# LiqunZhao/Neural-ordinary-differential-equations-based-Lyapunov-Barrier-Actor-Critic-NLBAC

Measured on AMD Instinct MI355X. Metric: ODE-integrate+update samples/sec, Unicycle batch 4096, higher is better.
Workload: dtype f32; 1 GPU; Unicycle B=4096 dopri5 (BASELINE.json configs[1] at B=4096 dopri5); NODE fit on 32768 rows every 10 updates; replay of 65536 synthetic transitions resident in HBM; solver=dopri5, adjoint=False, batch_per_gpu=4096, global_batch=4096, node_fit_rows_per_gpu=32768, parallelism=dp1, hipgraph=False

## Files before the change

include/nlbac_hip.h:

```cpp
#ifndef NLBAC_HIP_H
#define NLBAC_HIP_H

#ifdef __cplusplus
extern "C" {
#endif

#define NLBAC_ABI_VERSION 17
#define NLBAC_MAX_LAYERS 6
#define NLBAC_MAX_NETS 8
#define NLBAC_MLP_TILE 32

typedef void *nlbac_stream_t;

int nlbac_abi_version(void);
const char *nlbac_last_error(void);
int nlbac_elect_selftest(float *partials, unsigned *ticket, float *out, int n_blocks, int n_vals, unsigned salt,
                         nlbac_stream_t s);

typedef struct nlbac_mlp {
    int n_layers, in_dim, hid, out_dim;
    const float *params;
    int w_off[NLBAC_MAX_LAYERS];
    int b_off[NLBAC_MAX_LAYERS];
    float *packed;
    int pf_off[NLBAC_MAX_LAYERS];
    int pb_off[NLBAC_MAX_LAYERS];
    int rr_fwd_off, rr_bwd_off, packed_floats;
    int rr_kind;
} nlbac_mlp;

typedef struct nlbac_mlp_io {
    const float *x0; int x0_dim, x0_ld;
    const float *x1; int x1_dim, x1_ld;
    float *y; int y_ld;
    float *acts;
    long acts_ls;
    const float *dy; int dy_ld;
    int dz_first;
    float *dz;
    float *dx; int dx_ld;
    int dx_first;
    float *grad;
    float *skinny_ws;
    unsigned *masks;
} nlbac_mlp_io;

int nlbac_mlp_masks_ok(const nlbac_mlp *nets, int n_nets);

int nlbac_mlp_pack_layout(nlbac_mlp *net );
int nlbac_mlp_pack(const nlbac_mlp *nets, int n_nets, nlbac_stream_t s);

int nlbac_mlp_fwd(const nlbac_mlp *nets, const nlbac_mlp_io *io, int n_nets, int B, nlbac_stream_t s);
typedef struct nlbac_gauss_head {
    const float *eps, *scale, *bias; int n_u;
    float *action; int action_ld; float *logp;
    int cf_kind, cf_net, cf_nh;
    const float *cf_ps, *cf_ps_next, *cf_V, *cf_hazards;
    float cf_r2, cf_dt, cf_gamma_b, cf_gamma_l;
    float *cf_matr, *cf_bmatr, *cf_partials; unsigned *cf_tickets;
    int cf_n_cbf, cf_n_clf; float cf_batch_size; int cf_do_lambda_update, cf_do_backup_lambda_update, cf_ratio_mode, cf_backup_mode;
    float cf_lam_lo, cf_lam_hi;
    float *cf_sc;
    int cf_defer; unsigned *cf_tiles;
} nlbac_gauss_head;
int nlbac_mlp_fwd_gauss(const nlbac_mlp *nets, const nlbac_mlp_io *io, int n_nets, int B,
                        const nlbac_gauss_head *head, nlbac_stream_t s);
int nlbac_mlp_fwd_head_ok(const nlbac_mlp *nets, int n_nets);
int nlbac_mlp_fwd_head(const nlbac_mlp *nets, const nlbac_mlp_io *io, int n_nets, int B,
                       const nlbac_gauss_head *head, nlbac_stream_t s);
int nlbac_mlp_bwd_data(const nlbac_mlp *nets, const nlbac_mlp_io *io, int n_nets, int B, nlbac_stream_t s);
struct nlbac_dy_head;
int nlbac_mlp_bwd_data_head(const nlbac_mlp *nets, const nlbac_mlp_io *io, int n_nets, int B,
                            const struct nlbac_dy_head *head, nlbac_stream_t s);
long nlbac_mlp_bwd_weights_ws_floats(const nlbac_mlp *nets, int n_nets, int B);
int nlbac_mlp_bwd_weights(const nlbac_mlp *nets, const nlbac_mlp_io *io, int n_nets, int B,
                          int n_slabs, long slab_stride, float *ws, long ws_floats, nlbac_stream_t s);

int nlbac_adam_prepare(void *state, double lr, nlbac_stream_t s);
int nlbac_adam_step(float *p, float *m, float *v, const float *grad, int n_slabs, long slab_stride,
                    long n, const void *state, float *target, float tau, nlbac_stream_t s);
int nlbac_adam_fused(float *p, float *m, float *v, const float *grad, int n_slabs, long slab_stride, long n,
                     void *state, double lr, float *target, float tau, const void *scatter,
                     const void *scatter_target, int scatter_slots ,
                     int n_alpha ,
                     const long *alpha_off, float *const *alpha_dst,
                     const float *mirror_src, float *mirror_dst ,
                     int n_mirror, nlbac_stream_t s);
int nlbac_reduce_slabs(float *out, const float *grad, int n_slabs, long slab_stride, long n, nlbac_stream_t s);
int nlbac_soft_update(float *target, const float *src, long n, float tau, nlbac_stream_t s);

int nlbac_gauss_sample_fwd(const float *heads, int heads_ld, const float *eps, const float *scale,
                           const float *bias, int n_u, int n, float *action, int action_ld,
                           float *logp, nlbac_stream_t s);
int nlbac_gauss_sample_bwd(const float *heads, int heads_ld, const float *eps, const float *scale,
                           int n_u, int n, int rows_per_problem, const float *da0, int da0_ld,
                           const float *da1, int da1_ld, const float *da2, int da2_ld,
                           const float *alpha, float dlogp_mul, float *dheads, int dheads_ld,
                           nlbac_stream_t s);

#define NLBAC_SC_SIZE 128

int nlbac_td_targets(const float *q1t, const float *q2t, const float *lt, const float *nlogp,
                     const float *reward, const float *constraint, const float *mask, int rcm_ld,
                     const float *q1, const float *q2, const float *lf, const float *alpha,
                     float gamma, int B, int B_norm, float *dq1, float *dq2, float *dlf, float *next_q,
                     float *next_l, float *partials, unsigned *ticket, float mul, float *out, nlbac_stream_t s);

typedef struct nlbac_actor_scalar_args {
    float target_entropy;
    const float *log_alpha[2];
    float *g_log_alpha[2];
    float *sc;
} nlbac_actor_scalar_args;
int nlbac_actor_q_terms(const float *q1, const float *q2, const float *logp, const float *alpha,
                        int B, int B_norm, int P, float *dq1, float *dq2, float *partials,
                        const nlbac_actor_scalar_args *fused, unsigned *ticket, nlbac_stream_t s);
typedef struct nlbac_auglag_args {
    int n_cbf, n_clf;
    float batch_size;
    int do_lambda_update, do_backup_lambda_update, ratio_mode, backup_mode;
    float lam_lo, lam_hi;
} nlbac_auglag_args;
typedef struct nlbac_head_sums {
    int kind;
    int n_nets;
    const float *partials;
    const unsigned *n_tiles;
    float mul; float *out; float *out_x;
    int B_norm; nlbac_actor_scalar_args actor;
    float *sc;
} nlbac_head_sums;
typedef struct nlbac_dy_head {
    int kind, B_norm;
    const float *heads; int heads_ld; const float *eps; const float *scale; int n_u;
    const float *da[3]; int da_ld[3];
    const float *alpha;
    float dlogp_mul; float *dheads; int dheads_ld;
    const float *q1t, *q2t, *lt, *nlogp, *reward, *constraint, *mask; int rcm_ld;
    const float *q[3]; float gamma; float *dq[3]; float *next_q, *next_l;
    const float *xt, *xsig; int xsig_ld; const float *xq; float *dxq; float *out_x;
    const float *qa, *qb, *logp; float *dqa, *dqb; int n_prob;
    nlbac_actor_scalar_args actor;
    float *partials; unsigned *ticket; float mul; float *out;
    int cb_kind, cb_nh;
    const float *cb_ps_next, *cb_matr, *cb_bmatr, *cb_hazards, *cb_sc;
    float cb_dt, cb_batch;
    float *cb_dps_next, *cb_dV;
    int sums_defer; unsigned *sums_tiles;
    nlbac_head_sums finish[3];
    int cb_defer; const float *cb_partials; const unsigned *cb_tiles; nlbac_auglag_args cb_auglag; float *cb_stage;
} nlbac_dy_head;
int nlbac_actor_scalars(const float *partials, int n_blk, int B, int first_problem, int P, float target_entropy,
                        const float *log_alpha, int log_alpha_stride, float *g_log_alpha, float *sc,
                        nlbac_stream_t s);
int nlbac_alpha_refresh(const float *log_alpha, int log_alpha_stride, int first_problem, int P, float *sc,
                        nlbac_stream_t s);

int nlbac_unicycle_state(const float *obs, int obs_ld, int B, float l_p,
                         float *state ,
                         int n_copies, float *ps , nlbac_stream_t s);
int nlbac_unicycle_lookahead(const float *x , int n, float l_p, float *ps , nlbac_stream_t s);
int nlbac_unicycle_lookahead_bwd(const float *x, const float *dps, const float *dps2 , int n,
                                 float l_p, float *dx , nlbac_stream_t s);

int nlbac_unicycle_constraints_fwd(const float *ps, const float *ps_next, const float *V,
                                   const float *V_next, const float *hazards, int n_hz, float r_coll,
                                   float dt, float gamma_b, float gamma_l, int B, float *matr,
                                   float *bmatr, float *partials, const nlbac_auglag_args *fused,
                                   unsigned *ticket, float *sc, nlbac_stream_t s);
int nlbac_auglag(const float *partials, int n_blk, int n_cbf, int n_clf, float batch_size,
                 int do_lambda_update, int do_backup_lambda_update ,
                 int ratio_mode, int backup_mode, float lam_lo, float lam_hi, float *sc, nlbac_stream_t s);
int nlbac_unicycle_constraints_bwd(const float *ps_next, const float *matr, const float *bmatr,
                                   const float *hazards, int n_hz, float dt, float batch_size, int B,
                                   const float *sc, float *dps_next, float *dV_next, nlbac_stream_t s);

int nlbac_cars_state(const float *obs, int obs_ld, int n, float *state, nlbac_stream_t s);
int nlbac_cars_rollout_inputs(const float *mb, int ld, int t_col, int nt_col, const float *pi2, int B,
                              float *state, float *y0_2, float *c1, float *c2, nlbac_stream_t s);
int nlbac_cars_obs(const float *state, int n, float *obs, nlbac_stream_t s);
int nlbac_cars_constraints_fwd(const float *state, const float *x1, const float *x2, const float *V,
                               const float *V1, float gamma_b, float gamma_l, float radius, int B,
                               float *matr, float *bmatr, float *partials, const nlbac_auglag_args *fused,
                               unsigned *ticket, float *sc, nlbac_stream_t s);
int nlbac_cars_constraints_bwd(const float *matr, const float *bmatr, float gamma_b, float batch_size, int B,
                               const float *sc, float *dx1, float *dx2, float *dV1, nlbac_stream_t s);
int nlbac_add_cols(float *dst, int dst_ld, int col0, const float *src, int src_ld, int ncols, int n,
                   nlbac_stream_t s);
int nlbac_add_cols_plus(float *dst, int ld, int col0, const float *src, int src_ld, int ncols, int n_src,
                        const float *add, int n, nlbac_stream_t s);

int nlbac_td_value(const float *next_target, const float *signal, int sig_ld, const float *mask, int mask_ld,
                   const float *pred, float gamma, int B, int B_norm, float *dpred, float *next_out ,
                   float *partials, unsigned *ticket, float mul, float *out, nlbac_stream_t s);
int nlbac_unicycle_obs_fwd(const float *x , int n, float goal_x, float goal_y, float *obs, int obs_ld,
                           nlbac_stream_t s);
int nlbac_unicycle_obs_bwd(const float *x, const float *dobs, int dobs_ld, int n, float goal_x, float goal_y,
                           float *dx , int accumulate, nlbac_stream_t s);
int nlbac_barrier_constraints_fwd(const float *Bv, const float *Bn, const float *V, const float *Vn, float dt,
                                  float gamma_b, float gamma_l, int B, float *matr, float *partials,
                                  const nlbac_auglag_args *fused, unsigned *ticket, float *sc, nlbac_stream_t s);
int nlbac_barrier_constraints_bwd(const float *matr, float dt, float batch_size, int B, const float *sc,
                                  float *dBn, float *dVn, nlbac_stream_t s);

int nlbac_pvtol_state(const float *obs, int obs_ld, int n, float *st6, float *op , nlbac_stream_t s);
int nlbac_pvtol_obs_fwd(const float *x6, const float *op_prev, int op_rows, float follow, float goal_x, float goal_y,
                        int n, float *obs, int obs_ld, float *op_out , nlbac_stream_t s);
int nlbac_pvtol_obs_bwd(const float *x6, const float *dobs, int dobs_ld, float follow, float goal_x, float goal_y,
                        int n, float *dx, int accumulate, nlbac_stream_t s);
int nlbac_pvtol_constraints_fwd(const float *st6, const float *op0, const float *x1, const float *x2, const float *x3,
                                const float *V, const float *V1, const float *hazards, int n_hz, float r_coll,
                                float d_op, float y_max, float y_min, float follow, float gamma_b, float gamma_l,
                                int B, int NP, float *matr, float *bmatr, float *partials,
                                const nlbac_auglag_args *fused, unsigned *ticket, float *sc, nlbac_stream_t s);
int nlbac_pvtol_constraints_bwd(const float *matr, const float *bmatr, const float *x1, const float *x2,
                                const float *x3, const float *hazards, int n_hz, float follow, float gamma_b,
                                float batch_size, int B, int NP, const float *sc, float *dx1, float *dx2, float *dx3,
                                float *dV1, nlbac_stream_t s);

int nlbac_mse_fwd_bwd(const float *pred, int pred_ld, const float *target, int target_ld, int n, int n_norm,
                      int d, float *dpred, int dpred_ld, float *partials, nlbac_stream_t s);

int nlbac_affine_combine_fwd(const float *f, const float *g, const float *u, int n_s, int n_u, int n,
                             float *k, nlbac_stream_t s);
int nlbac_affine_combine_bwd(const float *dk, const float *g, const float *u, int n_s, int n_u, int n,
                             float mul, float *dg, float *du, int accumulate_du, nlbac_stream_t s);
int nlbac_rk_combine(const float *y0, const float *K, int n_k, const float *coef, const float *h_host,
                     const double *h_dev, int h_dev_stride, int P, int rows_per_problem, int n_s,
                     float *out, nlbac_stream_t s);
int nlbac_rk_stage_bwd(const float *dYup, const float *dXf, const float *dXg, int dx_ld, int n_k,
                       const float *coef, const float *h_host, const double *h_dev, int h_dev_stride,
                       int P, int rows_per_problem, int n_s, float *dK, float *dy0, int accumulate_dy0,
                       float *du_ext , int n_ext,
                       nlbac_stream_t s);
typedef struct nlbac_rk_chain {
    const double *ctl;
    long slot_floats;
    int norm_mode;
    int n_slots;
    float rtol, atol;
    double t_end;
    float *partials;
    unsigned *tickets;
    double *ctl_w;
    double *hslots;
    double *alog;
    int alog_cap;
    double *ctl_host;
    float *interp_out;
    int interp_kind; float interp_l; float *interp_p;
    int interp_bwd;
    const float *interp_dout, *interp_dp, *interp_dp2, *interp_x;
    double ctl_seq;
    int norm_defer, norm_pre;
    const float *partials_pre;
} nlbac_rk_chain;
int nlbac_rk_interp_ok(const nlbac_mlp *f, const nlbac_mlp *g);
typedef struct nlbac_in_map {
    int kind;
    const float *obs; int obs_ld;
    float l;
    float *ps;
} nlbac_in_map;
int nlbac_node_rk_fwd(const nlbac_mlp *f, const nlbac_mlp *g, const float *y0, const float *u, int P,
                      int rows_per_problem, int stage_begin, int stage_end, int n_stages_total,
                      const float *beta, const float *c_out, int n_out, const float *c_err, int n_err,
                      const float *h_host, const double *h_dev, int h_dev_stride, float *K, float *Y,
                      float *G, float *acts_f, long acts_f_ls, float *acts_g, long acts_g_ls, int acts_bits,
                      float *out, float *err, const nlbac_rk_chain *chain,
                      const nlbac_in_map *in_map , nlbac_stream_t s);
int nlbac_node_rk_mask_words(const nlbac_mlp *f, const nlbac_mlp *g, int which);
int nlbac_node_rk_bwd(const nlbac_mlp *f, const nlbac_mlp *g, const float *u, const float *G, int P,
                      int rows_per_problem, int n_stages_total, int st_lo, int st_hi, int dx_stage0,
                      const float *beta, const float *h_host, const double *h_dev, int h_dev_stride,
                      const float *acts_f, long acts_f_ls, const float *acts_g, long acts_g_ls,
                      int acts_bits ,
                      float *dz_f, float *dz_g, float *dG, float *dK, const float *dYup, float *dy0,
                      int dy0_in, float *du, int du_acc, const nlbac_rk_chain *chain, int back_idx,
                      nlbac_stream_t s);
int nlbac_node_rk_traj_ok(const nlbac_mlp *f, const nlbac_mlp *g);
int nlbac_node_rk_traj_fwd(const nlbac_mlp *f, const nlbac_mlp *g, const float *x0, const float *u, int n, int H,
                           int n_stages, const float *beta, const float *c_out, float h, float *out, float *K, float *Y,
                           float *G, float *acts_f, long acts_f_ls, float *acts_g, long acts_g_ls, int acts_bits,
                           nlbac_stream_t s);
int nlbac_node_rk_traj_bwd(const nlbac_mlp *f, const nlbac_mlp *g, const float *u, int n, int H, int n_stages,
                           const float *beta, const float *c_out, float h, const float *G, const float *acts_f,
                           long acts_f_ls, const float *acts_g, long acts_g_ls, int acts_bits, const float *dout,
                           float *dx0, float *du, float *dK, float *dG, float *dz_f, float *dz_g, nlbac_stream_t s);
int nlbac_concat_rk_traj_ok(const nlbac_mlp *net);
int nlbac_concat_rk_traj_fwd(const nlbac_mlp *net, const float *x0, const float *c, int n, int H, int n_stages,
                             const float *beta, const float *c_out, float h, float *out, float *Xin, float *acts,
                             long acts_ls, int acts_bits, const float *norm, nlbac_stream_t s);
int nlbac_concat_rk_traj_bwd(const nlbac_mlp *net, int n, int H, int n_stages, const float *beta, const float *c_out,
                             float h, const float *acts, long acts_ls, int acts_bits, const float *norm,
                             const float *dout, float *dx0, float *dc, float *dK, float *dz, nlbac_stream_t s);
int nlbac_node_rk_grid_fwd(const nlbac_mlp *f, const nlbac_mlp *g, const float *x0, const float *u, int n, int H,
                           int n_stages, const float *beta, const float *c_out, const float *hs, const float *hs_host,
                           float *out, float *K, float *Y, float *G, float *acts_f, long acts_f_ls, float *acts_g,
                           long acts_g_ls, int acts_bits, nlbac_stream_t s);
int nlbac_node_rk_grid_bwd(const nlbac_mlp *f, const nlbac_mlp *g, const float *u, int n, int H, int n_stages,
                           const float *beta, const float *c_out, const float *hs, const float *hs_host,
                           const float *G, const float *acts_f, long acts_f_ls, const float *acts_g, long acts_g_ls,
                           int acts_bits, const float *dout, float *dx0, float *du, float *dK, float *dG, float *dz_f,
                           float *dz_g, nlbac_stream_t s);
int nlbac_concat_rk_grid_fwd(const nlbac_mlp *net, const float *x0, const float *c, int n, int H, int n_stages,
                             const float *beta, const float *c_out, const float *hs, const float *hs_host, float *out,
                             float *Xin, float *acts, long acts_ls, int acts_bits, const float *norm, nlbac_stream_t s);
int nlbac_concat_rk_grid_bwd(const nlbac_mlp *net, int n, int H, int n_stages, const float *beta, const float *c_out,
                             const float *hs, const float *hs_host, const float *acts, long acts_ls, int acts_bits,
                             const float *norm, const float *dout, float *dx0, float *dc, float *dK, float *dz,
                             nlbac_stream_t s);
int nlbac_node_rk_subgrid_fwd(const nlbac_mlp *f, const nlbac_mlp *g, const float *x0, const float *u, int n, int H,
                              int n_stages, const float *beta, const float *c_out, const float *hs,
                              const float *hs_host, const int *ofs, const int *ofs_host, const float *theta,
                              const float *theta_host, int T, float *out, float *K, float *Y, float *G, float *acts_f,
                              long acts_f_ls, float *acts_g, long acts_g_ls, int acts_bits, nlbac_stream_t s);
int nlbac_node_rk_subgrid_bwd(const nlbac_mlp *f, const nlbac_mlp *g, const float *u, int n, int H, int n_stages,
                              const float *beta, const float *c_out, const float *hs, const float *hs_host,
                              const int *ofs, const int *ofs_host, const float *theta, const float *theta_host, int T,
                              const float *G, const float *acts_f, long acts_f_ls, const float *acts_g, long acts_g_ls,
                              int acts_bits, const float *dout, float *dx0, float *du, float *dK, float *dG,
                              float *dz_f, float *dz_g, nlbac_stream_t s);
int nlbac_concat_rk_subgrid_fwd(const nlbac_mlp *net, const float *x0, const float *c, int n, int H, int n_stages,
                                const float *beta, const float *c_out, const float *hs, const float *hs_host,
                                const int *ofs, const int *ofs_host, const float *theta, const float *theta_host, int T,
                                float *out, float *Xin, float *acts, long acts_ls, int acts_bits, const float *norm,
                                nlbac_stream_t s);
int nlbac_concat_rk_subgrid_bwd(const nlbac_mlp *net, int n, int H, int n_stages, const float *beta, const float *c_out,
                                const float *hs, const float *hs_host, const int *ofs, const int *ofs_host,
                                const float *theta, const float *theta_host, int T, const float *acts, long acts_ls,
                                int acts_bits, const float *norm, const float *dout, float *dx0, float *dc, float *dK,
                                float *dz, nlbac_stream_t s);
int nlbac_node_rk_hold_fwd(const nlbac_mlp *f, const nlbac_mlp *g, const float *x0, const float *u, int n, int H,
                           int n_stages, const float *beta, const float *c_out, const float *hs, const float *hs_host,
                           int m, float *out, float *K, float *Y, float *G, float *acts_f, long acts_f_ls,
                           float *acts_g, long acts_g_ls, int acts_bits, nlbac_stream_t s);
int nlbac_node_rk_hold_bwd(const nlbac_mlp *f, const nlbac_mlp *g, const float *u, int n, int H, int n_stages,
                           const float *beta, const float *c_out, const float *hs, const float *hs_host, int m,
                           const float *G, const float *acts_f, long acts_f_ls, const float *acts_g, long acts_g_ls,
                           int acts_bits, const float *dout, float *dx0, float *du, float *dK, float *dG, float *dz_f,
                           float *dz_g, nlbac_stream_t s);
int nlbac_concat_rk_hold_fwd(const nlbac_mlp *net, const float *x0, const float *c, int n, int H, int n_stages,
                             const float *beta, const float *c_out, const float *hs, const float *hs_host, int m,
                             float *out, float *Xin, float *acts, long acts_ls, int acts_bits, const float *norm,
                             nlbac_stream_t s);
int nlbac_concat_rk_hold_bwd(const nlbac_mlp *net, int n, int H, int n_stages, const float *beta, const float *c_out,
                             const float *hs, const float *hs_host, int m, const float *acts, long acts_ls,
                             int acts_bits, const float *norm, const float *dout, float *dx0, float *dc, float *dK,
                             float *dz, nlbac_stream_t s);
int nlbac_concat_rk_fwd(const nlbac_mlp *net, const float *y0, const float *c, int P, int rows_per_problem,
                        int stage_begin, int stage_end, int n_stages_total, const float *beta,
                        const float *c_out, int n_out, const float *c_err, int n_err, const float *h_host,
                        const double *h_dev, int h_dev_stride, float *K, float *Y, float *acts, long acts_ls,
                        int acts_bits ,
                        float *out, float *err, const float *norm, float *Xn, const struct nlbac_rk_chain *chain,
                        nlbac_stream_t s);
int nlbac_concat_rk_mask_words(const nlbac_mlp *net);
int nlbac_concat_rk_bwd(const nlbac_mlp *net, int P, int rows_per_problem, int n_stages_total, int st_lo,
                        int st_hi, int dx_stage0, const float *beta, const float *h_host, const double *h_dev,
                        int h_dev_stride, const float *acts, long acts_ls, int acts_bits , float *dz,
                        float *dK, const float *dYup,
                        float *dy0, int dy0_in, float *dc, int dc_acc, const float *norm, float *dyn,
                        const struct nlbac_rk_chain *chain, int back_idx, nlbac_stream_t s);
#define NLBAC_DOPRI_CTL 16
int nlbac_dopri_norm_partials(const float *a, const float *b, const float *y0, const float *y1,
                              const float *u, int mode, float rtol, float atol, int n_s, int n_u,
                              int rows_per_problem, int P, float *partials,
                              const double *slot_ctl ,
                              long slot_floats, nlbac_stream_t s);
int nlbac_dopri_norm_control(const float *a, const float *b, const float *y0, const float *y1, const float *u,
                             int mode, float rtol, float atol, int n_s, int n_u, int rows_per_problem, int P,
                             double t_end, float *partials, unsigned *tickets, double *ctl,
                             const struct nlbac_rk_chain *chain ,
                             nlbac_stream_t s);
int nlbac_dopri_control(const float *partials, int n_blk_per_problem, int mode, int n_s, int n_u,
                        int rows_per_problem, int P, double t_end, double *ctl,
                        int n_slots ,
                        double *hslots ,
                        double *alog , int alog_cap, nlbac_stream_t s);
int nlbac_dopri_control_tiles(const struct nlbac_rk_chain *chain, int n_s, int n_u, int rows_per_problem, int P,
                              nlbac_stream_t s);
typedef struct nlbac_out_map {
    int kind;
    float l;
    float *p;
    const float *dp, *dp2, *x;
} nlbac_out_map;
int nlbac_dopri_interp_fwd(const float *y0, const float *y1, const float *K, const float *h_host,
                           const float *x_host, const double *ctl, int P, int rows_per_problem, int n_s,
                           float *out, long slot_floats, const nlbac_out_map *map , nlbac_stream_t s);
int nlbac_dopri_interp_bwd(const float *dout, const float *h_host, const float *x_host, const double *ctl,
                           int P, int rows_per_problem, int n_s, float *dy0, float *dy1, float *dK,
                           long slot_floats, const nlbac_out_map *map , nlbac_stream_t s);

int nlbac_node_adj_step(const nlbac_mlp *f, const nlbac_mlp *g, const float *u, int P, int rows_per_problem,
                        int st_lo, int st_hi, int n_stages_total, const float *beta, const float *c_out, int n_out,
                        const float *c_err, int n_err, const float *h_host, const double *h_dev, int h_dev_stride,
                        const double *ctl, const float *Z0, float *KZ, float *Z1, float *ERR, float *ZS, float *dG,
                        float *acts_f, long acts_f_ls, float *acts_g, long acts_g_ls, float *dz_f, float *dz_g,
                        float *interp_out , double t_end, nlbac_stream_t s);
int nlbac_node_adj_interp_ok(const nlbac_mlp *f, const nlbac_mlp *g);
int nlbac_adj_pack(const float *y, const float *a_x, int n_s, int n_u, int n, float *Z, nlbac_stream_t s);
int nlbac_adj_unpack(const float *Z, int n_s, int n_u, int n, float *dy0, float *du, nlbac_stream_t s);
int nlbac_adj_norm_control(const float *a, const float *b, const float *Z0, const float *Z1, const float *u, int mode,
                           float rtol, float atol, int n_s, int n_u, int rows_per_problem, int P, double t_end,
                           const float *pnorm, float *partials, unsigned *tickets, double *ctl,
                           double *ctl_host ,
                           double host_seq ,
                           nlbac_stream_t s);
int nlbac_adj_control(const float *partials, int n_blk_per_problem, int mode, int n_s, int n_u, int rows_per_problem,
                      int P, double t_end, const float *pnorm, double *ctl, nlbac_stream_t s);
int nlbac_adj_commit(const double *ctl, int rows_per_problem, long n_rows, int w, float *dst0, const float *src0,
                     float *dst1, const float *src1, nlbac_stream_t s);
int nlbac_adj_param_norm(int mode, const float *th0, const float *K, long k_stride, int n_stages, const float *c_sol,
                         const float *c_err, const float *h_host, const double *h_dev, const int *seg_off,
                         const int *seg_len, int n_seg, float rtol, float atol, const double *ctl, float *th1,
                         float *pseg, unsigned *ticket, float *pnorm, nlbac_stream_t s);

int nlbac_concat_adj_in(const float *ZS, int w, const float *c, int n_s, int n_c, const float *norm, int n,
                        float *Xin, float *Ay, nlbac_stream_t s);
int nlbac_concat_adj_out(const float *fnet, const float *dX, int n_s, int n_c, const float *norm, int n, int w,
                         float *KZ, nlbac_stream_t s);
int nlbac_concat_adj_step_ok(const nlbac_mlp *net);
int nlbac_concat_adj_step(const nlbac_mlp *net, const float *c, int P, int rows_per_problem, int st_lo, int st_hi,
                          int n_stages_total, const float *beta, const float *c_out, int n_out, const float *c_err,
                          int n_err, const float *h_host, const double *h_dev, int h_dev_stride, const double *ctl,
                          const float *Z0, float *KZ, float *Z1, float *ERR, const float *norm, float *Xin, float *Ay,
                          float *acts, long acts_ls, float *dz, float *interp_out ,
                          double t_end, nlbac_stream_t s);

int nlbac_copy_blocks(const void *src, long src_stride, void *dst, long dst_stride, long block_len, long n_blocks,
                      nlbac_stream_t s);
int nlbac_gather_rows(const float *src, long src_rows, int ld, const long *idx, long n_rows, float *dst,
                      nlbac_stream_t s);
int nlbac_sample_rows(const float *src, long src_rows, int ld, long n_rows, float *dst, float *eps, long n_eps,
                      unsigned long long seed, unsigned long long draw, nlbac_stream_t s);

int nlbac_unicycle_env_step(int n, const double *params , int max_steps, const double *hazards,
                            int n_hz, const double *action , double *state , int *ep_step,
                            double *last_dist, double *obs , double *reward, double *constraint, double *signal,
                            double *center , double *next_center , int *done, double *info ,
                            nlbac_stream_t s);
int nlbac_pvtol_env_step(int n, const double *params , int max_steps,
                         const double *hazards, int n_hz, const double *action , double *state ,
                         int *ep_step, double *obs , double *reward, double *constraint, double *signal,
                         double *lya_pre , int *done, double *info,
                         nlbac_stream_t s);
int nlbac_cars_env_step(int n, const double *params ,
                        int max_steps, const double *action , double *state , double *t, int *ep_step,
                        double *obs , double *reward, double *constraint, double *lya_pre ,
                        double *lya_next , int *done, double *info, nlbac_stream_t s);

int nlbac_axpby(float a, const float *x, float b, const float *y , long n, float *out, nlbac_stream_t s);
int nlbac_fill(float *p, float v, long n, nlbac_stream_t s);
int nlbac_sum_partials(const float *partials, int n_blk, int n_cols, float mul, float *out, nlbac_stream_t s);

#ifdef __cplusplus
}
#endif
#endif
```

neural-ordinary-differential-equations-based-lyapunov-barrier-actor-critic-nlbac_amd/_lib.py:

```python
import ctypes as C
import os
import subprocess

_HERE = os.path.dirname(os.path.abspath(__file__))
LIB_PATH = os.environ.get("NLBAC_HIP_LIB") or os.path.join(_HERE, "lib", "libnlbac_hip.so")
CSRC = os.path.join(_HERE, "csrc")

MAX_LAYERS, MAX_NETS, MLP_TILE = 6, 8, 32
MLP_TILE_MIN = 16
SC_SIZE, DOPRI_CTL = 128, 16

c_float_p = C.POINTER(C.c_float)
c_double_p = C.POINTER(C.c_double)
c_int_p = C.POINTER(C.c_int)


class NlbacError(RuntimeError):
    pass


class Mlp(C.Structure):
    _fields_ = [("n_layers", C.c_int), ("in_dim", C.c_int), ("hid", C.c_int), ("out_dim", C.c_int),
                ("params", C.c_void_p),
                ("w_off", C.c_int * MAX_LAYERS), ("b_off", C.c_int * MAX_LAYERS),
                ("packed", C.c_void_p),
                ("pf_off", C.c_int * MAX_LAYERS), ("pb_off", C.c_int * MAX_LAYERS),
                ("rr_fwd_off", C.c_int), ("rr_bwd_off", C.c_int), ("packed_floats", C.c_int), ("rr_kind", C.c_int)]


class MlpIO(C.Structure):
    _fields_ = [("x0", C.c_void_p), ("x0_dim", C.c_int), ("x0_ld", C.c_int),
                ("x1", C.c_void_p), ("x1_dim", C.c_int), ("x1_ld", C.c_int),
                ("y", C.c_void_p), ("y_ld", C.c_int),
                ("acts", C.c_void_p), ("acts_ls", C.c_long),
                ("dy", C.c_void_p), ("dy_ld", C.c_int), ("dz_first", C.c_int),
                ("dz", C.c_void_p),
                ("dx", C.c_void_p), ("dx_ld", C.c_int), ("dx_first", C.c_int),
                ("grad", C.c_void_p),
                ("skinny_ws", C.c_void_p),
                ("masks", C.c_void_p)]


class AuglagArgs(C.Structure):
    _fields_ = [("n_cbf", C.c_int), ("n_clf", C.c_int), ("batch_size", C.c_float), ("do_lambda_update", C.c_int),
                ("do_backup_lambda_update", C.c_int), ("ratio_mode", C.c_int), ("backup_mode", C.c_int),
                ("lam_lo", C.c_float), ("lam_hi", C.c_float)]


class ActorScalarArgs(C.Structure):
    _fields_ = [("target_entropy", C.c_float), ("log_alpha", C.c_void_p * 2), ("g_log_alpha", C.c_void_p * 2),
                ("sc", C.c_void_p)]


class GaussHead(C.Structure):
    _fields_ = [("eps", C.c_void_p), ("scale", C.c_void_p), ("bias", C.c_void_p), ("n_u", C.c_int),
                ("action", C.c_void_p), ("action_ld", C.c_int), ("logp", C.c_void_p),
                ("cf_kind", C.c_int), ("cf_net", C.c_int), ("cf_nh", C.c_int),
                ("cf_ps", C.c_void_p), ("cf_ps_next", C.c_void_p), ("cf_V", C.c_void_p), ("cf_hazards", C.c_void_p),
                ("cf_r2", C.c_float), ("cf_dt", C.c_float), ("cf_gamma_b", C.c_float), ("cf_gamma_l", C.c_float),
                ("cf_matr", C.c_void_p), ("cf_bmatr", C.c_void_p), ("cf_partials", C.c_void_p), ("cf_tickets", C.c_void_p),
                ("cf_n_cbf", C.c_int), ("cf_n_clf", C.c_int), ("cf_batch_size", C.c_float),
                ("cf_do_lambda_update", C.c_int), ("cf_do_backup_lambda_update", C.c_int), ("cf_ratio_mode", C.c_int),
                ("cf_backup_mode", C.c_int), ("cf_lam_lo", C.c_float), ("cf_lam_hi", C.c_float), ("cf_sc", C.c_void_p),
                ("cf_defer", C.c_int), ("cf_tiles", C.c_void_p)]


class HeadSums(C.Structure):
    _fields_ = [("kind", C.c_int), ("n_nets", C.c_int), ("partials", C.c_void_p), ("n_tiles", C.c_void_p),
                ("mul", C.c_float), ("out", C.c_void_p), ("out_x", C.c_void_p), ("B_norm", C.c_int),
                ("actor", ActorScalarArgs), ("sc", C.c_void_p)]


class DyHead(C.Structure):
    _fields_ = [("kind", C.c_int), ("B_norm", C.c_int),
                ("heads", C.c_void_p), ("heads_ld", C.c_int), ("eps", C.c_void_p), ("scale", C.c_void_p), ("n_u", C.c_int),
                ("da", C.c_void_p * 3), ("da_ld", C.c_int * 3),
                ("alpha", C.c_void_p), ("dlogp_mul", C.c_float), ("dheads", C.c_void_p), ("dheads_ld", C.c_int),
                ("q1t", C.c_void_p), ("q2t", C.c_void_p), ("lt", C.c_void_p), ("nlogp", C.c_void_p), ("reward", C.c_void_p),
                ("constraint", C.c_void_p), ("mask", C.c_void_p), ("rcm_ld", C.c_int),
                ("q", C.c_void_p * 3), ("gamma", C.c_float), ("dq", C.c_void_p * 3), ("next_q", C.c_void_p),
                ("next_l", C.c_void_p),
                ("xt", C.c_void_p), ("xsig", C.c_void_p), ("xsig_ld", C.c_int), ("xq", C.c_void_p), ("dxq", C.c_void_p),
                ("out_x", C.c_void_p),
                ("qa", C.c_void_p), ("qb", C.c_void_p), ("logp", C.c_void_p), ("dqa", C.c_void_p), ("dqb", C.c_void_p),
                ("n_prob", C.c_int), ("actor", ActorScalarArgs),
                ("partials", C.c_void_p), ("ticket", C.c_void_p), ("mul", C.c_float), ("out", C.c_void_p),
                ("cb_kind", C.c_int), ("cb_nh", C.c_int), ("cb_ps_next", C.c_void_p), ("cb_matr", C.c_void_p),
                ("cb_bmatr", C.c_void_p), ("cb_hazards", C.c_void_p), ("cb_sc", C.c_void_p), ("cb_dt", C.c_float),
                ("cb_batch", C.c_float), ("cb_dps_next", C.c_void_p), ("cb_dV", C.c_void_p),
                ("sums_defer", C.c_int), ("sums_tiles", C.c_void_p), ("finish", HeadSums * 3),
                ("cb_defer", C.c_int), ("cb_partials", C.c_void_p), ("cb_tiles", C.c_void_p), ("cb_auglag", AuglagArgs),
                ("cb_stage", C.c_void_p)]


class RkChain(C.Structure):
    _fields_ = [("ctl", C.c_void_p), ("slot_floats", C.c_long), ("norm_mode", C.c_int), ("n_slots", C.c_int),
                ("rtol", C.c_float), ("atol", C.c_float), ("t_end", C.c_double), ("partials", C.c_void_p),
                ("tickets", C.c_void_p), ("ctl_w", C.c_void_p), ("hslots", C.c_void_p), ("alog", C.c_void_p),
                ("alog_cap", C.c_int), ("ctl_host", C.c_void_p),
                ("interp_out", C.c_void_p), ("interp_kind", C.c_int), ("interp_l", C.c_float), ("interp_p", C.c_void_p),
                ("interp_bwd", C.c_int), ("interp_dout", C.c_void_p), ("interp_dp", C.c_void_p),
                ("interp_dp2", C.c_void_p), ("interp_x", C.c_void_p), ("ctl_seq", C.c_double),
                ("norm_defer", C.c_int), ("norm_pre", C.c_int), ("partials_pre", C.c_void_p)]


class InMap(C.Structure):
    _fields_ = [("kind", C.c_int), ("obs", C.c_void_p), ("obs_ld", C.c_int), ("l", C.c_float), ("ps", C.c_void_p)]


class OutMap(C.Structure):
    _fields_ = [("kind", C.c_int), ("l", C.c_float), ("p", C.c_void_p), ("dp", C.c_void_p), ("dp2", C.c_void_p),
                ("x", C.c_void_p)]


_P, _I, _F, _D, _L = C.c_void_p, C.c_int, C.c_float, C.c_double, C.c_long

_PROTOS = {
    "nlbac_abi_version": [],
    "nlbac_last_error": [],
    "nlbac_elect_selftest": [_P, _P, _P, _I, _I, C.c_uint, _P],
    "nlbac_mlp_pack_layout": [C.POINTER(Mlp)],
    "nlbac_mlp_pack": [C.POINTER(Mlp), _I, _P],
    "nlbac_mlp_fwd": [C.POINTER(Mlp), C.POINTER(MlpIO), _I, _I, _P],
    "nlbac_mlp_fwd_gauss": [C.POINTER(Mlp), C.POINTER(MlpIO), _I, _I, C.POINTER(GaussHead), _P],
    "nlbac_mlp_masks_ok": [C.POINTER(Mlp), _I],
    "nlbac_mlp_fwd_head_ok": [C.POINTER(Mlp), _I],
    "nlbac_mlp_fwd_head": [C.POINTER(Mlp), C.POINTER(MlpIO), _I, _I, C.POINTER(GaussHead), _P],
    "nlbac_mlp_bwd_data": [C.POINTER(Mlp), C.POINTER(MlpIO), _I, _I, _P],
    "nlbac_mlp_bwd_data_head": [C.POINTER(Mlp), C.POINTER(MlpIO), _I, _I, C.POINTER(DyHead), _P],
    "nlbac_mlp_bwd_weights_ws_floats": [C.POINTER(Mlp), _I, _I],
    "nlbac_mlp_bwd_weights": [C.POINTER(Mlp), C.POINTER(MlpIO), _I, _I, _I, _L, _P, _L, _P],
    "nlbac_adam_prepare": [_P, _D, _P],
    "nlbac_adam_step": [_P, _P, _P, _P, _I, _L, _L, _P, _P, _F, _P],
    "nlbac_adam_fused": [_P, _P, _P, _P, _I, _L, _L, _P, _D, _P, _F, _P, _P, _I, _I, C.POINTER(C.c_long),
                         C.POINTER(C.c_void_p), _P, _P, _I, _P],
    "nlbac_node_rk_mask_words": [C.POINTER(Mlp), C.POINTER(Mlp), _I],
    "nlbac_concat_adj_in": [_P, _I, _P, _I, _I, _P, _I, _P, _P, _P],
    "nlbac_concat_adj_out": [_P, _P, _I, _I, _P, _I, _I, _P, _P],
    "nlbac_concat_adj_step_ok": [C.POINTER(Mlp)],
    "nlbac_rk_interp_ok": [C.POINTER(Mlp), C.POINTER(Mlp)],
    "nlbac_concat_adj_step": [C.POINTER(Mlp), _P, _I, _I, _I, _I, _I, _P, _P, _I, _P, _I, _P, _P, _I, _P, _P, _P, _P, _P,
                              _P, _P, _P, _P, _L, _P, _P, _D, _P],
    "nlbac_node_adj_interp_ok": [C.POINTER(Mlp), C.POINTER(Mlp)],
    "nlbac_reduce_slabs": [_P, _P, _I, _L, _L, _P],
    "nlbac_soft_update": [_P, _P, _L, _F, _P],
    "nlbac_gauss_sample_fwd": [_P, _I, _P, _P, _P, _I, _I, _P, _I, _P, _P],
    "nlbac_gauss_sample_bwd": [_P, _I, _P, _P, _I, _I, _I, _P, _I, _P, _I, _P, _I, _P, _F, _P, _I, _P],
    "nlbac_td_targets": [_P] * 7 + [_I] + [_P] * 4 + [_F, _I, _I] + [_P] * 6 + [_P, _F, _P, _P],
    "nlbac_actor_q_terms": [_P, _P, _P, _P, _I, _I, _I, _P, _P, _P, C.POINTER(ActorScalarArgs), _P, _P],
    "nlbac_actor_scalars": [_P, _I, _I, _I, _I, _F, _P, _I, _P, _P, _P],
    "nlbac_alpha_refresh": [_P, _I, _I, _I, _P, _P],
    "nlbac_unicycle_state": [_P, _I, _I, _F, _P, _I, _P, _P],
    "nlbac_unicycle_lookahead": [_P, _I, _F, _P, _P],
    "nlbac_unicycle_lookahead_bwd": [_P, _P, _P, _I, _F, _P, _P],
    "nlbac_unicycle_constraints_fwd": [_P, _P, _P, _P, _P, _I, _F, _F, _F, _F, _I, _P, _P, _P, C.POINTER(AuglagArgs), _P, _P, _P],
    "nlbac_auglag": [_P, _I, _I, _I, _F, _I, _I, _I, _I, _F, _F, _P, _P],
    "nlbac_unicycle_constraints_bwd": [_P, _P, _P, _P, _I, _F, _F, _I, _P, _P, _P, _P],
    "nlbac_mse_fwd_bwd": [_P, _I, _P, _I, _I, _I, _I, _P, _I, _P, _P],
    "nlbac_affine_combine_fwd": [_P, _P, _P, _I, _I, _I, _P, _P],
    "nlbac_affine_combine_bwd": [_P, _P, _P, _I, _I, _I, _F, _P, _P, _I, _P],
    "nlbac_rk_combine": [_P, _P, _I, c_float_p, c_float_p, _P, _I, _I, _I, _I, _P, _P],
    "nlbac_rk_stage_bwd": [_P, _P, _P, _I, _I, c_float_p, c_float_p, _P, _I, _I, _I, _I, _P, _P, _I, _P, _I, _P],
    "nlbac_cars_state": [_P, _I, _I, _P, _P],
    "nlbac_cars_rollout_inputs": [_P, _I, _I, _I, _P, _I, _P, _P, _P, _P, _P],
    "nlbac_cars_obs": [_P, _I, _P, _P],
    "nlbac_cars_constraints_fwd": [_P, _P, _P, _P, _P, _F, _F, _F, _I, _P, _P, _P, C.POINTER(AuglagArgs), _P, _P, _P],
    "nlbac_cars_constraints_bwd": [_P, _P, _F, _F, _I, _P, _P, _P, _P, _P],
    "nlbac_add_cols": [_P, _I, _I, _P, _I, _I, _I, _P],
    "nlbac_add_cols_plus": [_P, _I, _I, _P, _I, _I, _I, _P, _I, _P],
    "nlbac_pvtol_state": [_P, _I, _I, _P, _P, _P],
    "nlbac_pvtol_obs_fwd": [_P, _P, _I, _F, _F, _F, _I, _P, _I, _P, _P],
    "nlbac_pvtol_obs_bwd": [_P, _P, _I, _F, _F, _F, _I, _P, _I, _P],
    "nlbac_pvtol_constraints_fwd": [_P, _P, _P, _P, _P, _P, _P, _P, _I, _F, _F, _F, _F, _F, _F, _F, _I, _I, _P, _P, _P,
                                    C.POINTER(AuglagArgs), _P, _P, _P],
    "nlbac_pvtol_constraints_bwd": [_P, _P, _P, _P, _P, _P, _I, _F, _F, _F, _I, _I, _P, _P, _P, _P, _P, _P],
    "nlbac_copy_blocks": [_P, _L, _P, _L, _L, _L, _P],
    "nlbac_gather_rows": [_P, _L, _I, _P, _L, _P, _P],
    "nlbac_sample_rows": [_P, _L, _I, _L, _P, _P, _L, C.c_uint64, C.c_uint64, _P],
    "nlbac_td_value": [_P, _P, _I, _P, _I, _P, _F, _I, _I, _P, _P, _P, _P, _F, _P, _P],
    "nlbac_unicycle_obs_fwd": [_P, _I, _F, _F, _P, _I, _P],
    "nlbac_unicycle_obs_bwd": [_P, _P, _I, _I, _F, _F, _P, _I, _P],
    "nlbac_barrier_constraints_fwd": [_P, _P, _P, _P, _F, _F, _F, _I, _P, _P, C.POINTER(AuglagArgs), _P, _P, _P],
    "nlbac_barrier_constraints_bwd": [_P, _F, _F, _I, _P, _P, _P, _P],
    "nlbac_node_rk_fwd": [C.POINTER(Mlp), C.POINTER(Mlp), _P, _P, _I, _I, _I, _I, _I, c_float_p, c_float_p, _I,
                          c_float_p, _I, c_float_p, _P, _I, _P, _P, _P, _P, _L, _P, _L, _I, _P, _P, C.POINTER(RkChain),
                          C.POINTER(InMap), _P],
    "nlbac_node_rk_bwd": [C.POINTER(Mlp), C.POINTER(Mlp), _P, _P, _I, _I, _I, _I, _I, _I, c_float_p, c_float_p, _P, _I,
                          _P, _L, _P, _L, _I, _P, _P, _P, _P, _P, _P, _I, _P, _I, C.POINTER(RkChain), _I, _P],
    "nlbac_node_rk_traj_ok": [C.POINTER(Mlp), C.POINTER(Mlp)],
    "nlbac_node_rk_traj_fwd": [C.POINTER(Mlp), C.POINTER(Mlp), _P, _P, _I, _I, _I, c_float_p, c_float_p, _F, _P, _P, _P,
                               _P, _P, _L, _P, _L, _I, _P],
    "nlbac_node_rk_traj_bwd": [C.POINTER(Mlp), C.POINTER(Mlp), _P, _I, _I, _I, c_float_p, c_float_p, _F, _P, _P, _L, _P,
                               _L, _I, _P, _P, _P, _P, _P, _P, _P, _P],
    "nlbac_concat_rk_traj_ok": [C.POINTER(Mlp)],
    "nlbac_concat_rk_traj_fwd": [C.POINTER(Mlp), _P, _P, _I, _I, _I, c_float_p, c_float_p, _F, _P, _P, _P, _L, _I, _P, _P],
    "nlbac_concat_rk_traj_bwd": [C.POINTER(Mlp), _I, _I, _I, c_float_p, c_float_p, _F, _P, _L, _I, _P, _P, _P, _P, _P, _P,
                                 _P],
    "nlbac_node_rk_grid_fwd": [C.POINTER(Mlp), C.POINTER(Mlp), _P, _P, _I, _I, _I, c_float_p, c_float_p, _P, c_float_p, _P,
                               _P, _P, _P, _P, _L, _P, _L, _I, _P],
    "nlbac_node_rk_grid_bwd": [C.POINTER(Mlp), C.POINTER(Mlp), _P, _I, _I, _I, c_float_p, c_float_p, _P, c_float_p, _P, _P,
                               _L, _P, _L, _I, _P, _P, _P, _P, _P, _P, _P, _P],
    "nlbac_concat_rk_grid_fwd": [C.POINTER(Mlp), _P, _P, _I, _I, _I, c_float_p, c_float_p, _P, c_float_p, _P, _P, _P, _L,
                                 _I, _P, _P],
    "nlbac_concat_rk_grid_bwd": [C.POINTER(Mlp), _I, _I, _I, c_float_p, c_float_p, _P, c_float_p, _P, _L, _I, _P, _P, _P,
                                 _P, _P, _P, _P],
    "nlbac_node_rk_subgrid_fwd": [C.POINTER(Mlp), C.POINTER(Mlp), _P, _P, _I, _I, _I, c_float_p, c_float_p, _P, c_float_p,
                                  _P, c_int_p, _P, c_float_p, _I, _P, _P, _P, _P, _P, _L, _P, _L, _I, _P],
    "nlbac_node_rk_subgrid_bwd": [C.POINTER(Mlp), C.POINTER(Mlp), _P, _I, _I, _I, c_float_p, c_float_p, _P, c_float_p,
                                  _P, c_int_p, _P, c_float_p, _I, _P, _P, _L, _P, _L, _I, _P, _P, _P, _P, _P, _P, _P, _P],
    "nlbac_concat_rk_subgrid_fwd": [C.POINTER(Mlp), _P, _P, _I, _I, _I, c_float_p, c_float_p, _P, c_float_p, _P, c_int_p,
                                    _P, c_float_p, _I, _P, _P, _P, _L, _I, _P, _P],
    "nlbac_concat_rk_subgrid_bwd": [C.POINTER(Mlp), _I, _I, _I, c_float_p, c_float_p, _P, c_float_p, _P, c_int_p, _P,
                                    c_float_p, _I, _P, _L, _I, _P, _P, _P, _P, _P, _P, _P],
    "nlbac_node_rk_hold_fwd": [C.POINTER(Mlp), C.POINTER(Mlp), _P, _P, _I, _I, _I, c_float_p, c_float_p, _P, c_float_p, _I,
                               _P, _P, _P, _P, _P, _L, _P, _L, _I, _P],
    "nlbac_node_rk_hold_bwd": [C.POINTER(Mlp), C.POINTER(Mlp), _P, _I, _I, _I, c_float_p, c_float_p, _P, c_float_p, _I, _P,
                               _P, _L, _P, _L, _I, _P, _P, _P, _P, _P, _P, _P, _P],
    "nlbac_concat_rk_hold_fwd": [C.POINTER(Mlp), _P, _P, _I, _I, _I, c_float_p, c_float_p, _P, c_float_p, _I, _P, _P, _P,
                                 _L, _I, _P, _P],
    "nlbac_concat_rk_hold_bwd": [C.POINTER(Mlp), _I, _I, _I, c_float_p, c_float_p, _P, c_float_p, _I, _P, _L, _I, _P, _P,
                                 _P, _P, _P, _P, _P],
    "nlbac_concat_rk_fwd": [C.POINTER(Mlp), _P, _P, _I, _I, _I, _I, _I, c_float_p, c_float_p, _I, c_float_p, _I, c_float_p,
                            _P, _I, _P, _P, _P, _L, _I, _P, _P, _P, _P, C.POINTER(RkChain), _P],
    "nlbac_concat_rk_mask_words": [C.POINTER(Mlp)],
    "nlbac_concat_rk_bwd": [C.POINTER(Mlp), _I, _I, _I, _I, _I, _I, c_float_p, c_float_p, _P, _I, _P, _L, _I, _P, _P, _P, _P,
                            _I, _P, _I, _P, _P, C.POINTER(RkChain), _I, _P],
    "nlbac_node_adj_step": [C.POINTER(Mlp), C.POINTER(Mlp), _P, _I, _I, _I, _I, _I, c_float_p, c_float_p, _I, c_float_p,
                            _I, c_float_p, _P, _I, _P, _P, _P, _P, _P, _P, _P, _P, _L, _P, _L, _P, _P, _P, _D, _P],
    "nlbac_adj_pack": [_P, _P, _I, _I, _I, _P, _P],
    "nlbac_adj_unpack": [_P, _I, _I, _I, _P, _P, _P],
    "nlbac_adj_norm_control": [_P, _P, _P, _P, _P, _I, _F, _F, _I, _I, _I, _I, _D, _P, _P, _P, _P, _P, _D, _P],
    "nlbac_adj_control": [_P, _I, _I, _I, _I, _I, _I, _D, _P, _P, _P],
    "nlbac_adj_param_norm": [_I, _P, _P, _L, _I, c_float_p, c_float_p, c_float_p, _P, _P, _P, _I, _F, _F, _P, _P, _P, _P, _P,
                             _P],
    "nlbac_adj_commit": [_P, _I, _L, _I, _P, _P, _P, _P, _P],
    "nlbac_dopri_norm_partials": [_P, _P, _P, _P, _P, _I, _F, _F, _I, _I, _I, _I, _P, _P, _L, _P],
    "nlbac_dopri_norm_control": [_P, _P, _P, _P, _P, _I, _F, _F, _I, _I, _I, _I, _D, _P, _P, _P, C.POINTER(RkChain), _P],
    "nlbac_dopri_control": [_P, _I, _I, _I, _I, _I, _I, _D, _P, _I, _P, _P, _I, _P],
    "nlbac_dopri_control_tiles": [C.POINTER(RkChain), _I, _I, _I, _I, _P],
    "nlbac_dopri_interp_fwd": [_P, _P, _P, c_float_p, c_float_p, _P, _I, _I, _I, _P, _L, C.POINTER(OutMap), _P],
    "nlbac_dopri_interp_bwd": [_P, c_float_p, c_float_p, _P, _I, _I, _I, _P, _P, _P, _L, C.POINTER(OutMap), _P],
    "nlbac_unicycle_env_step": [_I, c_double_p, _I] + [_P, _I] + [_P] * 13,
    "nlbac_pvtol_env_step": [_I, c_double_p, _I] + [_P, _I] + [_P] * 11,
    "nlbac_cars_env_step": [_I, c_double_p, _I] + [_P] * 12,
    "nlbac_axpby": [_F, _P, _F, _P, _L, _P, _P],
    "nlbac_fill": [_P, _F, _L, _P],
    "nlbac_sum_partials": [_P, _I, _I, _F, _P, _P],
}
_RESTYPE = {"nlbac_last_error": C.c_char_p, "nlbac_mlp_bwd_weights_ws_floats": C.c_long}

EXPORTS = tuple(_PROTOS)

_lib = None


def build(verbose=False):
    r = subprocess.run(["make", "-C", CSRC, "-j4"], capture_output=True, text=True)
    if verbose or r.returncode != 0:
        print(r.stdout[-4000:])
        print(r.stderr[-4000:])
    if r.returncode != 0:
        raise NlbacError("hipcc build failed (see output above)")
    return LIB_PATH


ABI_VERSION = 17


def _stale_sources():
    try:
        t_lib = os.path.getmtime(LIB_PATH)
        header = os.path.join(os.path.dirname(_HERE), "include", "nlbac_hip.h")
        srcs = [os.path.join(CSRC, f) for f in os.listdir(CSRC) if f.endswith((".hip", ".h"))] + [header]
        return [os.path.basename(f) for f in srcs if os.path.exists(f) and os.path.getmtime(f) > t_lib + 1.0]
    except OSError:
        return []


def load():
    global _lib
    if _lib is not None:
        return _lib
    if not os.path.exists(LIB_PATH):
        raise NlbacError("HIP extension missing: %s (run __graft_entry__.build() / make -C %s); "
                         "there is no CPU fallback" % (LIB_PATH, CSRC))
    import torch
    lib = C.CDLL(LIB_PATH)
    for name, argtypes in _PROTOS.items():
        fn = getattr(lib, name)
        fn.argtypes = argtypes
        fn.restype = _RESTYPE.get(name, C.c_int)
    if lib.nlbac_abi_version() != ABI_VERSION:
        raise NlbacError("libnlbac_hip.so reports ABI version %d, this binding is written against %d: rebuild it "
                         "(make -C %s)" % (lib.nlbac_abi_version(), ABI_VERSION, CSRC))
    stale = _stale_sources()
    if stale:
        import warnings
        warnings.warn("libnlbac_hip.so is older than %s: rebuild it (make -C %s)" % (", ".join(stale), CSRC))
    _lib = lib
    return lib


def check(rc, what=""):
    if rc != 0:
        raise NlbacError("%s failed: %s" % (what, load().nlbac_last_error().decode()))


def call(name, *args):
    lib = load()
    rc = getattr(lib, name)(*args)
    if rc != 0:
        raise NlbacError("%s: %s" % (name, lib.nlbac_last_error().decode()))


def fptr(*vals):
    return (C.c_float * len(vals))(*vals)
```

neural-ordinary-differential-equations-based-lyapunov-barrier-actor-critic-nlbac_amd/arena.py:

```python
import ctypes as C

import torch

from . import _lib
from ._lib import MAX_LAYERS, Mlp, MlpIO


def _align4(n):
    return (n + 3) & ~3


class Arena:
    def __init__(self, device, n_slabs=8, with_target=False):
        self.device = torch.device(device)
        self.n_slabs = n_slabs
        self.with_target = with_target
        self._pending = []
        self.size = 0
        self.theta = None
        self.handles = []
        self._scatter = None

    def add_group(self, params):
        offs = []
        self.size = _align4(self.size)
        for p in params:
            offs.append(self.size)
            self._pending.append((p, self.size))
            self.size += p.numel()
        return offs

    def finalize(self):
        n = _align4(self.size)
        self.n = n
        dev = self.device
        self.theta = torch.zeros(n, dtype=torch.float32, device=dev)
        self.grad = torch.zeros(self.n_slabs, n, dtype=torch.float32, device=dev)
        self.m = torch.zeros(n, dtype=torch.float32, device=dev)
        self.v = torch.zeros(n, dtype=torch.float32, device=dev)
        self.target = torch.zeros(n, dtype=torch.float32, device=dev) if self.with_target else None
        self.state = torch.zeros(4, dtype=torch.int32, device=dev)
        self.offset_of = {}
        with torch.no_grad():
            for p, off in self._pending:
                view = self.theta[off:off + p.numel()].view(p.shape)
                view.copy_(p.data.to(dev))
                p.data = view
                self.offset_of[id(p)] = off
        return self

    def hard_update_target(self):
        self.target.copy_(self.theta)

    def scatter_tables(self):
        if self._scatter is not None:
            return self._scatter
        import numpy as np
        hs = [h for h in self.handles if h.desc is not None]
        n = self.n
        assert hs and n < (1 << 24), "index ramp must stay exact in fp32"
        keep = self.theta.clone()
        self.theta.copy_(torch.arange(1, n + 1, dtype=torch.float32))
        pack(hs)
        torch.cuda.synchronize()
        src_all, addr_all, addr_t_all = [], [], []
        for h in hs:
            pk = h.packed.cpu().numpy()
            slots = np.nonzero(pk)[0]
            src_all.append(pk[slots].astype(np.int64) - 1)
            addr_all.append(np.uint64(h.packed.data_ptr()) + slots.astype(np.uint64) * np.uint64(4))
            if self.with_target:
                addr_t_all.append(np.uint64(h.packed_target.data_ptr()) + slots.astype(np.uint64) * np.uint64(4))
        src = np.concatenate(src_all)
        order = np.argsort(src, kind="stable")
        src = src[order]
        start = np.ones(len(src), dtype=bool)
        start[1:] = src[1:] != src[:-1]
        first_idx = np.maximum.accumulate(np.where(start, np.arange(len(src)), 0))
        occ = np.arange(len(src)) - first_idx
        S = 2 if occ.max() < 2 else 4
        assert occ.max() < S, "a parameter has more than four fragment slots"

        def table(addrs):
            a = np.concatenate(addrs)[order]
            t = np.zeros((n, S), dtype=np.uint64)
            t[src, occ] = a
            return torch.from_numpy(t.view(np.int64).reshape(-1)).to(self.device)

        tab = table(addr_all)
        tab_t = table(addr_t_all) if self.with_target else None
        self.theta.copy_(keep)
        pack(hs)
        if self.with_target:
            pack(hs, target=True)
        th = self.theta.cpu().numpy()
        t_np = tab.cpu().numpy().view(np.uint64).reshape(n, S)
        for h in hs:
            pk = h.packed.cpu().numpy()
            base = np.uint64(h.packed.data_ptr())
            chk = np.zeros_like(pk)
            for c in range(S):
                a = t_np[:, c]
                sel = (a >= base) & (a < base + np.uint64(4 * pk.size))
                chk[((a[sel] - base) // np.uint64(4)).astype(np.int64)] = th[sel]
            assert np.array_equal(chk, pk), "scatter table does not reproduce nlbac_mlp_pack for %s" % h.name
        self.scatter_slots = S
        self._scatter = (tab, tab_t)
        return self._scatter

    def grad_view(self, p, slab=None):
        off = self.offset_of[id(p)]
        g = self.grad[:, off:off + p.numel()]
        return g.sum(0).view(p.shape) if slab is None else g[slab].view(p.shape)


class MlpHandle:

    def __init__(self, arena, layers, name=""):
        self.arena, self.name = arena, name
        self.layers = layers
        flat = []
        for W, b in layers:
            Ws = list(W) if isinstance(W, (list, tuple)) else [W]
            bs = list(b) if isinstance(b, (list, tuple)) else [b]
            flat.append((Ws, bs))
        self._flat = flat
        self.n_layers = len(flat)
        assert 2 <= self.n_layers <= MAX_LAYERS
        W0 = flat[0][0][0]
        self.in_dim, self.hid = W0.shape[1], W0.shape[0]
        self.out_dim = sum(w.shape[0] for w in flat[-1][0])
        for Ws, bs in flat:
            arena.add_group(Ws)
            arena.add_group(bs)
        arena.handles.append(self)
        self.desc = None
        self.desc_target = None

    def bind(self):
        a = self.arena
        d = Mlp()
        d.n_layers, d.in_dim, d.hid, d.out_dim = self.n_layers, self.in_dim, self.hid, self.out_dim
        for l, (Ws, bs) in enumerate(self._flat):
            d.w_off[l] = a.offset_of[id(Ws[0])]
            d.b_off[l] = a.offset_of[id(bs[0])]
        a._scatter = None
        lib = _lib.load()
        n_packed = lib.nlbac_mlp_pack_layout(C.byref(d))
        self.packed = torch.zeros(max(n_packed, 4), dtype=torch.float32, device=a.device)
        d.params = a.theta.data_ptr()
        d.packed = self.packed.data_ptr()
        self.desc = d
        if a.with_target:
            t = Mlp()
            C.memmove(C.byref(t), C.byref(d), C.sizeof(Mlp))
            self.packed_target = torch.zeros_like(self.packed)
            t.params = a.target.data_ptr()
            t.packed = self.packed_target.data_ptr()
            self.desc_target = t
        return self

    def params(self):
        out = []
        for Ws, bs in self._flat:
            out += Ws + bs
        return out


def mlp_array(descs):
    arr = (Mlp * len(descs))()
    for i, d in enumerate(descs):
        C.memmove(C.byref(arr, i * C.sizeof(Mlp)), C.byref(d), C.sizeof(Mlp))
    return arr


def io_array(n):
    return (MlpIO * n)()


def ptr(t):
    return t.data_ptr() if t is not None else None


_raw_stream = getattr(torch._C, "_cuda_getCurrentRawStream", None)


def stream_ptr():
    if _raw_stream is not None:
        return _raw_stream(torch.cuda.current_device())
    return torch.cuda.current_stream().cuda_stream


def pack(handles, target=False):
    cache = handles[0].__dict__.setdefault("_pack_cache", {})
    key = (tuple(id(h) for h in handles), target)
    arrs = cache.get(key)
    if arrs is None:
        if target == "both":
            descs = [h.desc for h in handles] + [h.desc_target for h in handles]
        else:
            descs = [h.desc_target if target else h.desc for h in handles]
        arrs = [(mlp_array(descs[i:i + _lib.MAX_NETS]), len(descs[i:i + _lib.MAX_NETS]))
                for i in range(0, len(descs), _lib.MAX_NETS)]
        cache[key] = (arrs, list(handles))
    else:
        arrs = arrs[0]
    s = stream_ptr()
    for arr, n in arrs:
        _lib.call("nlbac_mlp_pack", arr, n, s)


_BW_WS = {}


def skinny_partials_ws(nets, io_sets, n_nets, B, device):
    if B > 32768 or any(nets[i].hid > 256 for i in range(n_nets)):
        return None
    need = _lib.load().nlbac_mlp_bwd_weights_ws_floats(nets, n_nets, B)
    ws = torch.empty(max(need, 4), dtype=torch.float32, device=device)
    for i in range(n_nets):
        for io in io_sets:
            io[i].skinny_ws = ws.data_ptr() + 4 * i * (need // n_nets)
            io[i].dz_first = 1
    return ws


def bwd_weights(nets, io, n_nets, B, n_slabs, slab_stride, device, ws=None):
    lib = _lib.load()
    need = lib.nlbac_mlp_bwd_weights_ws_floats(nets, n_nets, B)
    key = str(device)
    if ws is None:
        ws = _BW_WS.get(key)
    if ws is None or ws.numel() < need:
        ws = torch.empty(max(need, 1 << 20), dtype=torch.float32, device=device)
        _BW_WS[key] = ws
    _lib.call("nlbac_mlp_bwd_weights", nets, io, n_nets, B, n_slabs, slab_stride, ws.data_ptr(), ws.numel(),
              stream_ptr())
```

neural-ordinary-differential-equations-based-lyapunov-barrier-actor-critic-nlbac_amd/csrc/optim_kernels.hip:

```cpp
#include <cstdint>
#include "common.h"

thread_local char nlbac_err_buf[512] = "";

extern "C" int nlbac_abi_version(void) { return NLBAC_ABI_VERSION; }
extern "C" const char* nlbac_last_error(void) { return nlbac_err_buf; }

struct AdamState {
    int step;
    float step_size;
    float bc2_sqrt;
    unsigned ticket;
};

__global__ void adam_prepare_kernel(AdamState* st, double lr) {
    if (threadIdx.x == 0 && blockIdx.x == 0) {
        const int t = st->step + 1;
        st->step = t;
        const double bc1 = 1.0 - pow(0.9, (double)t);
        const double bc2 = 1.0 - pow(0.999, (double)t);
        st->step_size = (float)(lr / bc1);
        st->bc2_sqrt = (float)sqrt(bc2);
    }
}

__device__ __forceinline__ float adam_one(float& p, float& m, float& v, float g, float step_size, float bc2_sqrt) {
    m = m + (g - m) * (float)(1.0 - 0.9);
    v = v * 0.999f + ((float)(1.0 - 0.999) * g) * g;
    const float denom = sqrtf(v) / bc2_sqrt + 1e-8f;
    p = p + ((-step_size) * m) / denom;
    return p;
}

__global__ __launch_bounds__(256) void adam_step_kernel(float* __restrict__ p, float* __restrict__ m,
                                                        float* __restrict__ v, const float* __restrict__ grad,
                                                        int n_slabs, long slab_stride, long n,
                                                        const AdamState* __restrict__ st,
                                                        float* __restrict__ target, float tau) {
    const float step_size = st->step_size, bc2_sqrt = st->bc2_sqrt;
    const long n4 = n >> 2;
    const long stride = (long)gridDim.x * blockDim.x;
    for (long i = (long)blockIdx.x * blockDim.x + threadIdx.x; i < n4; i += stride) {
        float4 g = reinterpret_cast<const float4*>(grad)[i];
        for (int s = 1; s < n_slabs; ++s) {
            const float4 gs = reinterpret_cast<const float4*>(grad + s * slab_stride)[i];
            g.x += gs.x; g.y += gs.y; g.z += gs.z; g.w += gs.w;
        }
        float4 pp = reinterpret_cast<float4*>(p)[i];
        float4 mm = reinterpret_cast<float4*>(m)[i];
        float4 vv = reinterpret_cast<float4*>(v)[i];
        adam_one(pp.x, mm.x, vv.x, g.x, step_size, bc2_sqrt);
        adam_one(pp.y, mm.y, vv.y, g.y, step_size, bc2_sqrt);
        adam_one(pp.z, mm.z, vv.z, g.z, step_size, bc2_sqrt);
        adam_one(pp.w, mm.w, vv.w, g.w, step_size, bc2_sqrt);
        reinterpret_cast<float4*>(p)[i] = pp;
        reinterpret_cast<float4*>(m)[i] = mm;
        reinterpret_cast<float4*>(v)[i] = vv;
        if (target) {
            float4 t = reinterpret_cast<float4*>(target)[i];
            t.x = t.x * (1.0f - tau) + pp.x * tau; t.y = t.y * (1.0f - tau) + pp.y * tau;
            t.z = t.z * (1.0f - tau) + pp.z * tau; t.w = t.w * (1.0f - tau) + pp.w * tau;
            reinterpret_cast<float4*>(target)[i] = t;
        }
    }
    for (long i = (n4 << 2) + (long)blockIdx.x * blockDim.x + threadIdx.x; i < n; i += stride) {
        float g = grad[i];
        for (int s = 1; s < n_slabs; ++s) g += grad[s * slab_stride + i];
        float pp = p[i], mm = m[i], vv = v[i];
        adam_one(pp, mm, vv, g, step_size, bc2_sqrt);
        p[i] = pp; m[i] = mm; v[i] = vv;
        if (target) target[i] = target[i] * (1.0f - tau) + pp * tau;
    }
}

template <int SLOTS>
__device__ __forceinline__ void scatter_n(const unsigned long long* __restrict__ scat, long i, float val) {
#pragma unroll
    for (int k = 0; k < SLOTS / 2; ++k) {
        const ulonglong2 ab = reinterpret_cast<const ulonglong2*>(scat)[i * (SLOTS / 2) + k];
        if (ab.x) *reinterpret_cast<float*>(ab.x) = val;
        if (ab.y) *reinterpret_cast<float*>(ab.y) = val;
    }
}
#define scatter2 scatter_n<SLOTS>

__device__ __forceinline__ float4 slab_sum4(const float* __restrict__ grad, int n_slabs, long slab_stride, long i) {
    float4 g = reinterpret_cast<const float4*>(grad)[i];
    int s = 1;
    for (; s + 3 < n_slabs; s += 4) {
        const float4 a = reinterpret_cast<const float4*>(grad + (long)s * slab_stride)[i];
        const float4 b = reinterpret_cast<const float4*>(grad + (long)(s + 1) * slab_stride)[i];
        const float4 c = reinterpret_cast<const float4*>(grad + (long)(s + 2) * slab_stride)[i];
        const float4 d = reinterpret_cast<const float4*>(grad + (long)(s + 3) * slab_stride)[i];
        g.x += a.x; g.y += a.y; g.z += a.z; g.w += a.w;
        g.x += b.x; g.y += b.y; g.z += b.z; g.w += b.w;
        g.x += c.x; g.y += c.y; g.z += c.z; g.w += c.w;
        g.x += d.x; g.y += d.y; g.z += d.z; g.w += d.w;
    }
    for (; s < n_slabs; ++s) {
        const float4 a = reinterpret_cast<const float4*>(grad + (long)s * slab_stride)[i];
        g.x += a.x; g.y += a.y; g.z += a.z; g.w += a.w;
    }
    return g;
}

struct AlphaRefresh { long off[2]; float* dst[2]; const float* mirror_src; float* mirror_dst; int n_mirror; };
__device__ __forceinline__ void alpha_refresh(const AlphaRefresh& AR, long e, float p_new) {
#pragma unroll
    for (int k = 0; k < 2; ++k)
        if (e == AR.off[k]) {
            const float a = expf(p_new);
            *AR.dst[k] = a;
            if (AR.mirror_dst) {
                const long i = AR.dst[k] - AR.mirror_src;
                if (i >= 0 && i < AR.n_mirror) AR.mirror_dst[i] = a;
            }
        }
}

template <int SLOTS>
__global__ __launch_bounds__(256) void adam_fused_kernel(float* __restrict__ p, float* __restrict__ m,
                                                         float* __restrict__ v, const float* __restrict__ grad,
                                                         int n_slabs, long slab_stride, long n, AdamState* st, double lr,
                                                         float* __restrict__ target, float tau,
                                                         const unsigned long long* __restrict__ scat,
                                                         const unsigned long long* __restrict__ scat_t,
                                                         const AlphaRefresh AR) {
    __shared__ float s_const[2];
    __shared__ int s_step;
    if (threadIdx.x == 0) {
        const int t = __hip_atomic_load(&st->step, __ATOMIC_RELAXED, __HIP_MEMORY_SCOPE_AGENT) + 1;
        const double bc1 = 1.0 - pow(0.9, (double)t);
        const double bc2 = 1.0 - pow(0.999, (double)t);
        s_const[0] = (float)(lr / bc1);
        s_const[1] = (float)sqrt(bc2);
        s_step = t;
    }
    __syncthreads();
    const float step_size = s_const[0], bc2_sqrt = s_const[1];
    const long n4 = n >> 2;
    const long stride = (long)gridDim.x * blockDim.x;
    for (long i = (long)blockIdx.x * blockDim.x + threadIdx.x; i < n4; i += stride) {
        float4 g = slab_sum4(grad, n_slabs, slab_stride, i);
        float4 pp = reinterpret_cast<float4*>(p)[i];
        float4 mm = reinterpret_cast<float4*>(m)[i];
        float4 vv = reinterpret_cast<float4*>(v)[i];
        adam_one(pp.x, mm.x, vv.x, g.x, step_size, bc2_sqrt);
        adam_one(pp.y, mm.y, vv.y, g.y, step_size, bc2_sqrt);
        adam_one(pp.z, mm.z, vv.z, g.z, step_size, bc2_sqrt);
        adam_one(pp.w, mm.w, vv.w, g.w, step_size, bc2_sqrt);
        reinterpret_cast<float4*>(p)[i] = pp;
        reinterpret_cast<float4*>(m)[i] = mm;
        reinterpret_cast<float4*>(v)[i] = vv;
        if (AR.off[0] >= 0 || AR.off[1] >= 0) {
            alpha_refresh(AR, 4 * i + 0, pp.x); alpha_refresh(AR, 4 * i + 1, pp.y);
            alpha_refresh(AR, 4 * i + 2, pp.z); alpha_refresh(AR, 4 * i + 3, pp.w);
        }
        if (scat) {
            scatter2(scat, 4 * i + 0, pp.x); scatter2(scat, 4 * i + 1, pp.y);
            scatter2(scat, 4 * i + 2, pp.z); scatter2(scat, 4 * i + 3, pp.w);
        }
        if (target) {
            float4 t = reinterpret_cast<float4*>(target)[i];
            t.x = t.x * (1.0f - tau) + pp.x * tau; t.y = t.y * (1.0f - tau) + pp.y * tau;
            t.z = t.z * (1.0f - tau) + pp.z * tau; t.w = t.w * (1.0f - tau) + pp.w * tau;
            reinterpret_cast<float4*>(target)[i] = t;
            if (scat_t) {
                scatter2(scat_t, 4 * i + 0, t.x); scatter2(scat_t, 4 * i + 1, t.y);
                scatter2(scat_t, 4 * i + 2, t.z); scatter2(scat_t, 4 * i + 3, t.w);
            }
        }
    }
    for (long i = (n4 << 2) + (long)blockIdx.x * blockDim.x + threadIdx.x; i < n; i += stride) {
        float g = grad[i];
        for (int s = 1; s < n_slabs; ++s) g += grad[s * slab_stride + i];
        float pp = p[i], mm = m[i], vv = v[i];
        adam_one(pp, mm, vv, g, step_size, bc2_sqrt);
        p[i] = pp; m[i] = mm; v[i] = vv;
        alpha_refresh(AR, i, pp);
        if (scat) scatter2(scat, i, pp);
        if (target) {
            const float t = target[i] * (1.0f - tau) + pp * tau;
            target[i] = t;
            if (scat_t) scatter2(scat_t, i, t);
        }
    }
    __syncthreads();
    __shared__ int s_is_last;
    if (threadIdx.x == 0) {
        s_is_last = 0;
        const unsigned ticket = __hip_atomic_fetch_add(&st->ticket, 1u, __ATOMIC_RELAXED, __HIP_MEMORY_SCOPE_AGENT);
        if (ticket == gridDim.x - 1) {
            __hip_atomic_store(&st->ticket, 0u, __ATOMIC_RELAXED, __HIP_MEMORY_SCOPE_AGENT);
            st->step_size = step_size;
            st->bc2_sqrt = bc2_sqrt;
            __hip_atomic_store(&st->step, s_step, __ATOMIC_RELAXED, __HIP_MEMORY_SCOPE_AGENT);
            s_is_last = 1;
        }
    }
    if (!AR.mirror_dst) return;
    __syncthreads();
    if (s_is_last)
        for (int i = threadIdx.x; i < AR.n_mirror; i += blockDim.x) {
            const bool refreshed = (AR.off[0] >= 0 && AR.dst[0] == AR.mirror_src + i) ||
                                   (AR.off[1] >= 0 && AR.dst[1] == AR.mirror_src + i);
            if (!refreshed) AR.mirror_dst[i] = AR.mirror_src[i];
        }
}

__global__ __launch_bounds__(256) void reduce_slabs_kernel(float* __restrict__ out, const float* __restrict__ grad,
                                                           int n_slabs, long slab_stride, long n) {
    const long stride = (long)gridDim.x * blockDim.x;
    for (long i = (long)blockIdx.x * blockDim.x + threadIdx.x; i < n; i += stride) {
        float g = grad[i];
        for (int s = 1; s < n_slabs; ++s) g += grad[s * slab_stride + i];
        out[i] = g;
    }
}

__global__ __launch_bounds__(256) void soft_update_kernel(float* __restrict__ target, const float* __restrict__ src,
                                                          long n, float tau) {
    const long stride = (long)gridDim.x * blockDim.x;
    for (long i = (long)blockIdx.x * blockDim.x + threadIdx.x; i < n; i += stride)
        target[i] = target[i] * (1.0f - tau) + src[i] * tau;
}

__global__ __launch_bounds__(256) void axpby_kernel(float a, const float* x, float b, const float* y, long n, float* out) {
    const long stride = (long)gridDim.x * blockDim.x;
    for (long i = (long)blockIdx.x * blockDim.x + threadIdx.x; i < n; i += stride)
        out[i] = a * x[i] + (y ? b * y[i] : 0.f);
}

__global__ __launch_bounds__(256) void fill_kernel(float* p, float v, long n) {
    const long stride = (long)gridDim.x * blockDim.x;
    for (long i = (long)blockIdx.x * blockDim.x + threadIdx.x; i < n; i += stride) p[i] = v;
}

__global__ void sum_partials_kernel(const float* partials, int n_blk, int n_cols, float mul, float* out) {
    const int c = blockIdx.x * blockDim.x + threadIdx.x;
    if (c >= n_cols) return;
    float s = 0.f;
    for (int b = 0; b < n_blk; ++b) s += partials[(long)b * n_cols + c];
    out[c] = s * mul;
}

static inline int stream_grid(long n, int per_thread = 1) {
    long b = (n / per_thread + 255) / 256;
    if (b < 1) b = 1;
    if (b > 2048) b = 2048;
    return (int)b;
}

extern "C" int nlbac_adam_prepare(void* state, double lr, nlbac_stream_t s) {
    NLBAC_REQUIRE(state, "nlbac_adam_prepare: null state");
    hipLaunchKernelGGL(adam_prepare_kernel, dim3(1), dim3(64), 0, (hipStream_t)s, (AdamState*)state, lr);
    NLBAC_CHECK_LAUNCH("nlbac_adam_prepare");
    return 0;
}

extern "C" int nlbac_adam_step(float* p, float* m, float* v, const float* grad, int n_slabs, long slab_stride,
                               long n, const void* state, float* target, float tau, nlbac_stream_t s) {
    NLBAC_REQUIRE(p && m && v && grad && state, "nlbac_adam_step: null pointer");
    NLBAC_REQUIRE(n_slabs >= 1 && n >= 1, "nlbac_adam_step: bad sizes");
    NLBAC_REQUIRE(((uintptr_t)p | (uintptr_t)m | (uintptr_t)v | (uintptr_t)grad | (uintptr_t)target) % 16 == 0 &&
                      slab_stride % 4 == 0,
                  "nlbac_adam_step: buffers must be 16-byte aligned");
    hipLaunchKernelGGL(adam_step_kernel, dim3(stream_grid(n, 4)), dim3(256), 0, (hipStream_t)s, p, m, v, grad,
                       n_slabs, slab_stride, n, (const AdamState*)state, (tau >= 0.f) ? target : nullptr, tau);
    NLBAC_CHECK_LAUNCH("nlbac_adam_step");
    return 0;
}

extern "C" int nlbac_adam_fused(float* p, float* m, float* v, const float* grad, int n_slabs, long slab_stride, long n,
                                void* state, double lr, float* target, float tau, const void* scatter,
                                const void* scatter_target, int scatter_slots, int n_alpha, const long* alpha_off,
                                float* const* alpha_dst, const float* mirror_src, float* mirror_dst, int n_mirror,
                                nlbac_stream_t s) {
    NLBAC_REQUIRE(p && m && v && grad && state, "nlbac_adam_fused: null pointer");
    NLBAC_REQUIRE(scatter_slots == 2 || scatter_slots == 4 || (!scatter && !scatter_target),
                  "nlbac_adam_fused: scatter tables hold 2 or 4 slots per parameter");
    NLBAC_REQUIRE(n_alpha >= 0 && n_alpha <= 2 && (n_alpha == 0 || (alpha_off && alpha_dst)), "nlbac_adam_fused: bad alpha refresh");
    AlphaRefresh AR;
    AR.off[0] = AR.off[1] = -1; AR.dst[0] = AR.dst[1] = nullptr;
    NLBAC_REQUIRE((mirror_dst == nullptr) || (mirror_src && n_mirror > 0 && n_mirror <= 1024), "nlbac_adam_fused: bad mirror");
    AR.mirror_src = mirror_src; AR.mirror_dst = mirror_dst; AR.n_mirror = mirror_dst ? n_mirror : 0;
    for (int k = 0; k < n_alpha; ++k) {
        NLBAC_REQUIRE(alpha_off[k] >= 0 && alpha_off[k] < n && alpha_dst[k], "nlbac_adam_fused: alpha entry out of range");
        AR.off[k] = alpha_off[k]; AR.dst[k] = alpha_dst[k];
    }
    NLBAC_REQUIRE(n_slabs >= 1 && n >= 1 && lr > 0.0, "nlbac_adam_fused: bad sizes");
    NLBAC_REQUIRE(((uintptr_t)p | (uintptr_t)m | (uintptr_t)v | (uintptr_t)grad | (uintptr_t)target) % 16 == 0 &&
                      slab_stride % 4 == 0 && ((uintptr_t)scatter | (uintptr_t)scatter_target) % 8 == 0,
                  "nlbac_adam_fused: buffers must be 16-byte aligned");
    NLBAC_REQUIRE(!scatter_target || (target && tau >= 0.f), "nlbac_adam_fused: scatter_target without a target");
    hipLaunchKernelGGL((scatter_slots == 4 ? adam_fused_kernel<4> : adam_fused_kernel<2>), dim3(stream_grid(n, 4)), dim3(256),
                       0, (hipStream_t)s, p, m, v, grad, n_slabs, slab_stride, n, (AdamState*)state, lr,
                       (tau >= 0.f) ? target : nullptr, tau, (const unsigned long long*)scatter,
                       (const unsigned long long*)scatter_target, AR);
    NLBAC_CHECK_LAUNCH("nlbac_adam_fused");
    return 0;
}

extern "C" int nlbac_reduce_slabs(float* out, const float* grad, int n_slabs, long slab_stride, long n, nlbac_stream_t s) {
    NLBAC_REQUIRE(out && grad && n_slabs >= 1, "nlbac_reduce_slabs: bad arguments");
    hipLaunchKernelGGL(reduce_slabs_kernel, dim3(stream_grid(n)), dim3(256), 0, (hipStream_t)s, out, grad, n_slabs, slab_stride, n);
    NLBAC_CHECK_LAUNCH("nlbac_reduce_slabs");
    return 0;
}

extern "C" int nlbac_soft_update(float* target, const float* src, long n, float tau, nlbac_stream_t s) {
    NLBAC_REQUIRE(target && src, "nlbac_soft_update: null pointer");
    hipLaunchKernelGGL(soft_update_kernel, dim3(stream_grid(n)), dim3(256), 0, (hipStream_t)s, target, src, n, tau);
    NLBAC_CHECK_LAUNCH("nlbac_soft_update");
    return 0;
}

extern "C" int nlbac_axpby(float a, const float* x, float b, const float* y, long n, float* out, nlbac_stream_t s) {
    NLBAC_REQUIRE(x && out, "nlbac_axpby: null pointer");
    hipLaunchKernelGGL(axpby_kernel, dim3(stream_grid(n)), dim3(256), 0, (hipStream_t)s, a, x, b, y, n, out);
    NLBAC_CHECK_LAUNCH("nlbac_axpby");
    return 0;
}

extern "C" int nlbac_fill(float* p, float v, long n, nlbac_stream_t s) {
    NLBAC_REQUIRE(p, "nlbac_fill: null pointer");
    hipLaunchKernelGGL(fill_kernel, dim3(stream_grid(n)), dim3(256), 0, (hipStream_t)s, p, v, n);
    NLBAC_CHECK_LAUNCH("nlbac_fill");
    return 0;
}

extern "C" int nlbac_sum_partials(const float* partials, int n_blk, int n_cols, float mul, float* out, nlbac_stream_t s) {
    NLBAC_REQUIRE(partials && out && n_blk >= 1 && n_cols >= 1, "nlbac_sum_partials: bad arguments");
    hipLaunchKernelGGL(sum_partials_kernel, dim3(nlbac_ceil_div(n_cols, 64)), dim3(64), 0, (hipStream_t)s, partials, n_blk, n_cols, mul, out);
    NLBAC_CHECK_LAUNCH("nlbac_sum_partials");
    return 0;
}


__global__ __launch_bounds__(256) void gather_rows_kernel(const float4* __restrict__ src, int ld4,
                                                          const long* __restrict__ idx, long n_rows, long src_rows,
                                                          float4* __restrict__ dst) {
    const long t = (long)blockIdx.x * 256 + threadIdx.x;
    if (t >= n_rows * ld4) return;
    const long r = t / ld4;
    const int c = (int)(t - r * ld4);
    long j = idx[r];
    j = j < 0 ? 0 : (j >= src_rows ? src_rows - 1 : j);
    dst[r * ld4 + c] = src[j * ld4 + c];
}

__device__ __forceinline__ uint4 philox4x32_10(uint4 ctr, uint2 key) {
#pragma unroll
    for (int r = 0; r < 10; ++r) {
        const unsigned long long p0 = (unsigned long long)0xD2511F53u * ctr.x;
        const unsigned long long p1 = (unsigned long long)0xCD9E8D57u * ctr.z;
        ctr = make_uint4((unsigned)(p1 >> 32) ^ ctr.y ^ key.x, (unsigned)p1, (unsigned)(p0 >> 32) ^ ctr.w ^ key.y,
                         (unsigned)p0);
        key.x += 0x9E3779B9u;
        key.y += 0xBB67AE85u;
    }
    return ctr;
}

__device__ __forceinline__ float u01(unsigned x) { return (float)(x >> 8) * 0x1p-24f + 0x1p-25f; }

__global__ __launch_bounds__(256) void sample_rows_kernel(const float4* __restrict__ src, int ld4, long n_rows,
                                                          long src_rows, float4* __restrict__ dst,
                                                          float* __restrict__ eps, long n_eps,
                                                          unsigned long long seed, unsigned long long draw) {
    const long t = (long)blockIdx.x * 256 + threadIdx.x;
    const uint2 key = make_uint2((unsigned)seed, (unsigned)(seed >> 32));
    if (t < n_rows * ld4) {
        const long r = t / ld4;
        const int c = (int)(t - r * ld4);
        const uint4 x = philox4x32_10(make_uint4((unsigned)draw, (unsigned)(draw >> 32), (unsigned)r, 0u), key);
        const long j = (long)(((unsigned long long)x.x * (unsigned long long)src_rows) >> 32);
        dst[r * ld4 + c] = src[j * ld4 + c];
    }
    const long q = (n_eps + 3) >> 2;
    if (eps && t < q) {
        const uint4 x = philox4x32_10(make_uint4((unsigned)draw, (unsigned)(draw >> 32), (unsigned)t, 1u), key);
        const float r0 = sqrtf(-2.f * logf(u01(x.x))), r1 = sqrtf(-2.f * logf(u01(x.z)));
        float s0, c0, s1, c1;
        sincosf(6.283185307179586f * u01(x.y), &s0, &c0);
        sincosf(6.283185307179586f * u01(x.w), &s1, &c1);
        const float v[4] = {r0 * c0, r0 * s0, r1 * c1, r1 * s1};
        for (int k = 0; k < 4; ++k)
            if (4 * t + k < n_eps) eps[4 * t + k] = v[k];
    }
}

extern "C" int nlbac_sample_rows(const float* src, long src_rows, int ld, long n_rows, float* dst, float* eps,
                                 long n_eps, unsigned long long seed, unsigned long long draw, nlbac_stream_t s) {
    NLBAC_REQUIRE(src && dst && src_rows >= 1 && src_rows < (1L << 32) && n_rows >= 1 && n_eps >= 0,
                  "nlbac_sample_rows: bad arguments");
    NLBAC_REQUIRE(ld >= 4 && ld % 4 == 0 && ((uintptr_t)src % 16) == 0 && ((uintptr_t)dst % 16) == 0,
                  "nlbac_sample_rows: rows must be whole float4s (ld %d)", ld);
    NLBAC_REQUIRE(eps || n_eps == 0, "nlbac_sample_rows: n_eps without a buffer");
    const long total = n_rows * (ld / 4), q = (n_eps + 3) / 4;
    const long threads = total > q ? total : q;
    hipLaunchKernelGGL(sample_rows_kernel, dim3((unsigned)((threads + 255) / 256)), dim3(256), 0, (hipStream_t)s,
                       (const float4*)src, ld / 4, n_rows, src_rows, (float4*)dst, eps, n_eps, seed, draw);
    NLBAC_CHECK_LAUNCH("nlbac_sample_rows");
    return 0;
}

__global__ __launch_bounds__(256) void copy_blocks_kernel(const float* __restrict__ src, long src_stride,
                                                          float* __restrict__ dst, long dst_stride, long block_len,
                                                          long n_blocks) {
    const long total = block_len * n_blocks, stride = (long)gridDim.x * 256;
    for (long i = (long)blockIdx.x * 256 + threadIdx.x; i < total; i += stride) {
        const long b = i / block_len, j = i - b * block_len;
        dst[b * dst_stride + j] = src[b * src_stride + j];
    }
}

extern "C" int nlbac_copy_blocks(const void* src, long src_stride, void* dst, long dst_stride, long block_len,
                                 long n_blocks, nlbac_stream_t s) {
    NLBAC_REQUIRE(src && dst && block_len >= 1 && n_blocks >= 1 && src_stride >= block_len && dst_stride >= block_len,
                  "nlbac_copy_blocks: bad arguments");
    hipLaunchKernelGGL(copy_blocks_kernel, dim3(stream_grid(block_len * n_blocks)), dim3(256), 0, (hipStream_t)s,
                       (const float*)src, src_stride, (float*)dst, dst_stride, block_len, n_blocks);
    NLBAC_CHECK_LAUNCH("nlbac_copy_blocks");
    return 0;
}

extern "C" int nlbac_gather_rows(const float* src, long src_rows, int ld, const long* idx, long n_rows, float* dst,
                                 nlbac_stream_t s) {
    NLBAC_REQUIRE(src && idx && dst && src_rows >= 1 && n_rows >= 1, "nlbac_gather_rows: bad arguments");
    NLBAC_REQUIRE(ld >= 4 && ld % 4 == 0 && ((uintptr_t)src % 16) == 0 && ((uintptr_t)dst % 16) == 0,
                  "nlbac_gather_rows: rows must be whole float4s (ld %d)", ld);
    const long total = n_rows * (ld / 4);
    hipLaunchKernelGGL(gather_rows_kernel, dim3((unsigned)((total + 255) / 256)), dim3(256), 0, (hipStream_t)s,
                       (const float4*)src, ld / 4, idx, n_rows, src_rows, (float4*)dst);
    NLBAC_CHECK_LAUNCH("nlbac_gather_rows");
    return 0;
}
```

neural-ordinary-differential-equations-based-lyapunov-barrier-actor-critic-nlbac_amd/sac_cbf_clf/replay_memory.py:

```python
import random

import numpy as np

_FIELDS = ("state", "action", "reward", "constraint", "center_pos", "next_center_pos",
           "next_state", "mask", "t", "next_t")


class ReplayMemory:

    def __init__(self, capacity, seed, initial_rows=65536):
        random.seed(seed)
        self.capacity = int(capacity)
        self._rows = min(self.capacity, int(initial_rows))
        self._cols = None
        self._len = 0
        self.position = 0

    def _alloc(self, values):
        self._cols = []
        for v in values:
            a = np.asarray(0.0 if v is None else v, dtype=np.float64)
            self._cols.append(np.zeros((self._rows,) + a.shape, dtype=np.float64))

    def _grow(self):
        new_rows = min(self.capacity, self._rows * 2)
        self._cols = [np.concatenate([c, np.zeros((new_rows - self._rows,) + c.shape[1:])]) for c in self._cols]
        self._rows = new_rows

    def push(self, state, action, reward, constraint, center_pos, next_center_pos, next_state, mask,
             t=None, next_t=None):
        self._push((state, action, reward, constraint, center_pos, next_center_pos, next_state, mask, t, next_t))

    def _push(self, values):
        if self._cols is None:
            self._alloc(values)
        if self.position >= self._rows:
            self._grow()
        for c, v in zip(self._cols, values):
            c[self.position] = 0.0 if v is None else v
        self._len = max(self._len, self.position + 1)
        self.position = (self.position + 1) % self.capacity

    def sample(self, batch_size):
        idx = np.asarray(random.sample(range(self._len), batch_size), dtype=np.int64)
        return tuple(c[idx] for c in self._cols)

    def __len__(self):
        return self._len



class DeviceReplayMemory:

    def __init__(self, capacity, seed, agent, chunk=4096, device_rng=False):
        import torch
        random.seed(seed)
        self.capacity, self.agent, self.device_rng = int(capacity), agent, device_rng
        self.lay, self.device = agent.lay, agent.device
        self.n_fields = 11 if self.lay.sig is not None else 10
        self.rows = torch.zeros(self.capacity, self.lay.LD, dtype=torch.float32, device=self.device)
        self._stage = torch.zeros(min(chunk, self.capacity), self.lay.LD, dtype=torch.float32).pin_memory() \
            if torch.cuda.is_available() else torch.zeros(min(chunk, self.capacity), self.lay.LD)
        self._stage_np = self._stage.numpy()
        self._n_staged, self._stage_start = 0, 0
        self._len = 0
        self.position = 0
        self._seed = (int(seed) * 0x9E3779B97F4A7C15 + 0x632BE59BD9B4E019) & 0xFFFFFFFFFFFFFFFF
        self._draws = 0

    def push(self, *fields, t=None, next_t=None):
        fields = tuple(fields)
        if len(fields) == self.n_fields - 2:
            fields = fields + (t, next_t)
        assert len(fields) == self.n_fields, "push takes %d fields" % self.n_fields
        if self._n_staged == self._stage_np.shape[0] or \
                (self._n_staged and self._stage_start + self._n_staged != self.position):
            self.flush()
        if self._n_staged == 0:
            self._stage_start = self.position
        batch1 = tuple(np.asarray(0.0 if f is None else f, dtype=np.float64)[None] for f in fields)
        self._stage_np[self._n_staged] = self.agent._rows_from_host(batch1).numpy()[0]
        self._n_staged += 1
        self._len = max(self._len, self.position + 1)
        self.position = (self.position + 1) % self.capacity
        if self.position == 0:
            self.flush()

    def push_rows(self, rows):
        import torch
        self.flush()
        rows = torch.as_tensor(rows, dtype=torch.float32)
        n = rows.shape[0]
        assert rows.shape[1] == self.lay.LD and n <= self.capacity
        first = min(n, self.capacity - self.position)
        self.rows[self.position:self.position + first].copy_(rows[:first])
        if n > first:
            self.rows[:n - first].copy_(rows[first:])
        self._len = min(self.capacity, max(self._len, self.position + n))
        self.position = (self.position + n) % self.capacity

    def flush(self):
        if self._n_staged:
            self.rows[self._stage_start:self._stage_start + self._n_staged].copy_(self._stage[:self._n_staged],
                                                                                 non_blocking=False)
            self._n_staged = 0

    def sample_rows(self, batch_size, out=None, eps_out=None):
        import torch
        from .. import _lib
        from ..arena import stream_ptr
        self.flush()
        if out is None:
            out = torch.empty(batch_size, self.lay.LD, dtype=torch.float32, device=self.device)
        if self.device_rng:
            self._draws += 1
            _lib.call("nlbac_sample_rows", self.rows.data_ptr(), self._len, self.lay.LD, batch_size, out.data_ptr(),
                      eps_out.data_ptr() if eps_out is not None else None,
                      eps_out.numel() if eps_out is not None else 0, self._seed, self._draws, stream_ptr())
            return out
        idx = torch.tensor(random.sample(range(self._len), batch_size), dtype=torch.int64).to(self.device)
        _lib.call("nlbac_gather_rows", self.rows.data_ptr(), self._len, self.lay.LD, idx.data_ptr(), batch_size,
                  out.data_ptr(), stream_ptr())
        if eps_out is not None:
            eps_out.normal_()
        return out

    def sample(self, batch_size):
        rows = self.sample_rows(batch_size).cpu().numpy().astype(np.float64)
        lay = self.lay
        cols = [("obs", lay.obs_dim), ("act", lay.act_dim), ("rew", 0), ("con", 0)]
        if lay.sig is not None:
            cols.append(("sig", 0))
        cols += [("lya", lay.lya_dim), ("nlya", lay.lya_dim), ("nobs", lay.obs_dim), ("mask", 0), ("t", 0), ("nt", 0)]
        out = []
        for name, w in cols:
            c = getattr(lay, name)
            out.append(rows[:, c] if w == 0 else rows[:, c:c + w])
        return tuple(out)

    def __len__(self):
        return self._len
```

neural-ordinary-differential-equations-based-lyapunov-barrier-actor-critic-nlbac_amd/sac_cbf_clf/sac_cbf_clf.py:

```python
import collections
import ctypes as C
import os
import random
import types

import numpy as np
import torch
import torch.nn as nn

from .. import _lib
from ..arena import Arena, bwd_weights, pack, stream_ptr
from . import _layout as SC
from .model import BarrierNetwork, GaussianPolicy, LyaNetwork, QNetwork
from .scalars_readback import ScalarsReadback
from .tasks import TASKS
from .update_plan import GraphCache, Plan, _Layout, _Workspace
from .utils import to_tensor

DYNAMICS_MODE = {'Unicycle': {'n_s': 3, 'n_u': 2}, 'SimulatedCars': {'n_s': 10, 'n_u': 1},
                 'Pvtol': {'n_s': 6, 'n_u': 2}, 'Quadrotor': {'n_s': 6, 'n_u': 2}}
l_p = 0.03


class PoseLoss(nn.Module):

    def forward(self, predicted_state, true_state):
        return nn.functional.mse_loss(predicted_state, true_state)


class SAC_CBF_CLF(object):
    variant = ""

    def __init__(self, num_inputs, action_space, env, args):
        self.gamma = args.gamma
        self.gamma_b = args.gamma_b
        self.tau = args.tau
        self.policy_type = args.policy
        self.batch_size = args.batch_size
        self.target_update_interval = args.target_update_interval
        self.Lagrangian_multiplier_update_interval = args.Lagrangian_multiplier_update_interval
        self.automatic_entropy_tuning = args.automatic_entropy_tuning
        self.action_space = action_space
        self.action_space.seed(args.seed)
        if not args.cuda or not torch.cuda.is_available():
            raise RuntimeError("nlbac_amd.SAC_CBF_CLF runs on an MI355X only (pass --cuda on a GPU box); "
                               "there is no CPU fallback")
        if self.policy_type != "Gaussian":
            raise NotImplementedError("only the Gaussian policy is on the device path")
        if env.dynamics_mode + self.variant not in TASKS:
            raise Exception('Dynamics mode not supported.')
        _lib.load()
        self.device = torch.device("cuda")
        self.env = env
        self.task = task = TASKS[env.dynamics_mode + self.variant](self, env, args)
        self.lay = _Layout(task)
        if num_inputs != task.obs_dim or action_space.shape[0] != task.act_dim:
            raise ValueError("%s expects %d observations / %d actions" % (task.name, task.obs_dim, task.act_dim))
        self.center_pos_num = task.lya_dim
        self.critic_lyapunov_lr = 0.0004
        self.lr = args.lr
        hidden = args.hidden_size
        n_act = action_space.shape[0]
        self.num_inputs, self.n_act, self.hidden = num_inputs, n_act, hidden
        self.n_grad_slabs = int(getattr(args, "grad_slabs", 16 if int(getattr(args, "batch_size", 0) or 0) >= 16384 else 8))
        if os.environ.get("NLBAC_GRAD_SLABS"):
            self.n_grad_slabs = int(os.environ["NLBAC_GRAD_SLABS"])

        self.critic = QNetwork(num_inputs, n_act, hidden)
        self.lyapunovNet = LyaNetwork(self.center_pos_num, hidden)
        self.BarrierNet = BarrierNetwork(num_inputs, n_act, hidden) if task.has_signal else None
        QNetwork(num_inputs, n_act, hidden)
        LyaNetwork(self.center_pos_num, hidden)
        if task.has_signal:
            BarrierNetwork(num_inputs, n_act, hidden)
        self.cost_limit = 0.0
        self.augmented_ratio = 1.0005
        if args.seed >= 0:
            env.seed(args.seed)
            random.seed(args.seed)
            env.action_space.seed(args.seed)
            torch.manual_seed(args.seed)
            np.random.seed(args.seed)
            torch.cuda.manual_seed_all(args.seed)
        self.target_entropy = -float(np.prod(action_space.shape))
        self.log_alpha = nn.Parameter(torch.zeros(1))
        self.backup_log_alpha = nn.Parameter(torch.zeros(1))
        self.policy = GaussianPolicy(num_inputs, n_act, hidden, action_space)
        self.backup_policy = GaussianPolicy(num_inputs, n_act, hidden, action_space) if task.n_pol == 2 else None

        self.num_cbfs = task.num_cbfs
        self.l_p = l_p
        self.action_dim = env.action_space.shape[0]
        self.u_min, self.u_max = self.get_control_bounds()
        self.num_constraints = self.num_cbfs + 1
        self.neural_ode_model = task.build_node()
        self.solver = 'euler'
        self.model_loss_func = PoseLoss()
        self.atol, self.rtol = 1e-7, 1e-5

        dev = self.device
        self.ar_c = Arena(dev, self.n_grad_slabs, with_target=True)
        self.ar_a = Arena(dev, self.n_grad_slabs)
        self.n_fit_slabs = int(getattr(args, "fit_grad_slabs", 51))
        self.ar_n = Arena(dev, self.n_fit_slabs * 2)
        self.h_q1, self.h_q2 = self.critic.attach(self.ar_c)
        (self.h_l,) = self.lyapunovNet.attach(self.ar_c)
        self.h_extra = list(self.BarrierNet.attach(self.ar_c)) if task.has_signal else []
        (self.h_p,) = self.policy.attach(self.ar_a)
        self.h_pols = [self.h_p]
        self.ar_b = Arena(dev, self.n_grad_slabs) if (task.n_pol == 2 and task.backup_interval > 1) else None
        ar_backup = self.ar_b if self.ar_b is not None else self.ar_a
        if task.n_pol == 2:
            (self.h_b,) = self.backup_policy.attach(ar_backup)
            self.h_pols.append(self.h_b)
        self.ar_a.add_group([self.log_alpha])
        if task.n_pol == 2:
            ar_backup.add_group([self.backup_log_alpha])
        self.h_node = list(self.neural_ode_model.attach(self.ar_n))
        self.arenas = [a for a in (self.ar_c, self.ar_a, self.ar_b, self.ar_n) if a is not None]
        for ar in self.arenas:
            ar.finalize()
        self.ar_c.hard_update_target()
        self.policy.to(dev)
        if self.backup_policy is not None:
            self.backup_policy.to(dev)
        self.h_crit = [self.h_q1, self.h_q2, self.h_l] + self.h_extra
        for h in self.h_crit + self.h_pols + self.h_node:
            h.bind()
        la_off = self.ar_a.offset_of[id(self.log_alpha)]
        G = types.SimpleNamespace
        if self.ar_b is not None:
            self.actor_groups = [G(arena=self.ar_a, first=0, count=1, la_off=la_off, la_stride=0),
                                 G(arena=self.ar_b, first=1, count=1, la_stride=0,
                                   la_off=self.ar_b.offset_of[id(self.backup_log_alpha)])]
        else:
            stride = (self.ar_a.offset_of[id(self.backup_log_alpha)] - la_off) if task.n_pol == 2 else 0
            self.actor_groups = [G(arena=self.ar_a, first=0, count=task.n_pol, la_off=la_off, la_stride=stride)]
        self.pol_arena = [self.ar_a] + ([ar_backup] if task.n_pol == 2 else [])
        self.critic_target = _TargetView(self.critic, self.ar_c)
        self.lyapunovNet_target = _TargetView(self.lyapunovNet, self.ar_c)
        if task.has_signal:
            self.BarrierNet_target = _TargetView(self.BarrierNet, self.ar_c)
        self.repack_all()
        for ar in self.arenas:
            ar.scatter_tables()

        self.sc = torch.zeros(SC.SC_SIZE, dtype=torch.float32, device=dev)
        sc_host = np.zeros(SC.SC_SIZE, dtype=np.float32)
        sc_host[SC.SC_ALPHA] = sc_host[SC.SC_BALPHA] = args.alpha
        sc_host[SC.SC_RHO_F64:SC.SC_RHO_F64 + 2] = np.array([1.0], dtype=np.float64).view(np.float32)
        sc_host[SC.SC_BRHO_F64:SC.SC_BRHO_F64 + 2] = np.array([1.0], dtype=np.float64).view(np.float32)
        self.sc.copy_(torch.from_numpy(sc_host))
        task.setup()
        self._tickets = torch.zeros(16, dtype=torch.int32, device=dev)
        self._ws = {}
        self._noise = None
        self._fit_ws = {}
        self._fill = collections.deque()
        self._fill_first = True
        self._readback = ScalarsReadback(self.sc)
        for sv in self.task.solvers:
            sv.before_wait = self._fill_one
        self.use_graphs = False
        self.fold_launches = os.environ.get("NLBAC_FOLD", "1") != "0"
        self.sums_defer = os.environ.get("NLBAC_SUMS_DEFER", "1") != "0"
        self.adjoint = bool(getattr(args, "adjoint", False))
        self.dp = None
        self._xb = {}

    @property
    def adjoint(self):
        return self._adjoint

    @adjoint.setter
    def adjoint(self, on):
        self._adjoint = bool(on)
        for sv in self.task.solvers:
            sv.adjoint = bool(on)

    def _graphs_on(self):
        return self.use_graphs and self.world == 1 and self.task.graph_ok and not (self._adjoint and self.solver == "dopri5")

    @property
    def node_solver(self):
        return self.task.solvers[0]

    @property
    def fit_solver(self):
        return self.task.fit_solver

    def enable_data_parallel(self, dist, group=None, always_collective=False, step_control="global"):
        from ..parallel import DataParallel
        assert step_control in ("global", "shard")
        self.dp = DataParallel(dist, group, always_collective)
        self.dp_step_control = step_control
        for ar in self.arenas:
            self.dp.broadcast_(ar.theta)
        self.ar_c.hard_update_target()
        self.dp.broadcast_(self.sc)
        self.repack_all()
        for sv in self.task.solvers:
            sv.comm = self.dp if step_control == "global" else None
        return self

    @property
    def world(self):
        return self.dp.world if self.dp is not None else 1

    def _exchange_buf(self, name, n):
        if name not in self._xb:
            self._xb[name] = torch.zeros(n, dtype=torch.float32, device=self.device)
        return self._xb[name]

    def _adam(self, arena, lr, n_slabs, extra=None, target=None, tau=-1.0, before_step=None, alpha=None, mirror=None):
        s = stream_ptr()
        a = arena
        scat, scat_t = a.scatter_tables()
        scat_t = scat_t.data_ptr() if (scat_t is not None and target is not None and tau >= 0) else None
        n_al = len(alpha[0]) if alpha else 0
        al_off = (C.c_long * 2)(*(list(alpha[0]) + [0, 0])[:2]) if alpha else None
        al_dst = (C.c_void_p * 2)(*(list(alpha[1]) + [None, None])[:2]) if alpha else None
        if self.world == 1:
            if before_step is not None:
                before_step(a.grad.data_ptr())
            _lib.call("nlbac_adam_fused", a.theta.data_ptr(), a.m.data_ptr(), a.v.data_ptr(), a.grad.data_ptr(),
                      n_slabs, a.n, a.n, a.state.data_ptr(), lr, target, tau, scat.data_ptr(), scat_t, a.scatter_slots,
                      n_al, al_off, al_dst, self.sc.data_ptr() if mirror is not None else None,
                      mirror.data_ptr() if mirror is not None else None, SC.SC_SIZE if mirror is not None else 0, s)
            return
        n_extra = 0 if extra is None else extra.numel()
        xb = self._exchange_buf("g%d" % id(a), a.n + 4)
        _lib.call("nlbac_reduce_slabs", xb.data_ptr(), a.grad.data_ptr(), n_slabs, a.n, a.n, s)
        if n_extra:
            xb[a.n:a.n + n_extra].copy_(extra)
        self.dp.all_reduce_(xb)
        if n_extra:
            extra.copy_(xb[a.n:a.n + n_extra])
        if before_step is not None:
            before_step(xb.data_ptr())
        _lib.call("nlbac_adam_fused", a.theta.data_ptr(), a.m.data_ptr(), a.v.data_ptr(), xb.data_ptr(), 1, a.n, a.n,
                  a.state.data_ptr(), lr, target, tau, scat.data_ptr(), scat_t, a.scatter_slots, n_al, al_off, al_dst, None,
                  None, 0, s)

    def repack_all(self):
        pack(self.h_crit + self.h_pols + self.h_node)
        pack(self.h_crit, target=True)

    def set_noise(self, eps_list):
        self._noise = [torch.as_tensor(e, dtype=torch.float32) for e in eps_list]

    def _scalars(self):
        return self._readback.read()

    @property
    def alpha(self):
        return float(self._scalars()[SC.SC_ALPHA])

    @property
    def backup_alpha(self):
        return float(self._scalars()[SC.SC_BALPHA])

    @property
    def lambda_values(self):
        return [float(x) for x in self._scalars()[SC.SC_LAMBDA:SC.SC_LAMBDA + self.num_constraints]]

    @property
    def backup_lambda_values(self):
        return [float(x) for x in self._scalars()[SC.SC_BLAMBDA:SC.SC_BLAMBDA + self.num_cbfs]]

    @property
    def augmented_term(self):
        return float(self._scalars()[SC.SC_RHO_F64:SC.SC_RHO_F64 + 2].view(np.float64)[0])

    @property
    def backup_augmented_term(self):
        return float(self._scalars()[SC.SC_BRHO_F64:SC.SC_BRHO_F64 + 2].view(np.float64)[0])

    def get_control_bounds(self):
        u_min = torch.tensor(self.env.safe_action_space.low).to(self.device)
        u_max = torch.tensor(self.env.safe_action_space.high).to(self.device)
        return u_min, u_max

    def _select(self, policy, state, evaluate, warmup):
        if not warmup and np.ndim(state) == 1:
            return policy.act(np.asarray(state, dtype=np.float64), evaluate)
        state = to_tensor(np.asarray(state, dtype=np.float64), torch.FloatTensor, self.device)
        expand_dim = len(state.shape) == 1
        if expand_dim:
            state = state.unsqueeze(0)
        if warmup:
            action = torch.stack([torch.from_numpy(self.action_space.sample()) for _ in range(state.shape[0])])
        else:
            a, _, mean = policy.sample(state)
            action = mean if evaluate else a
        action = action.detach().cpu().numpy()
        return action[0] if expand_dim else action

    def select_action(self, state, evaluate=False, warmup=False):
        return self._select(self.policy, state, evaluate, warmup)

    def select_action_backup(self, state, evaluate=False, warmup=False):
        if self.backup_policy is None:
            raise AttributeError("this variant has no backup controller")
        return self._select(self.backup_policy, state, evaluate, warmup)

    def update_parameters(self, memory, batch_size, updates, dynamics_model, NODE_memory, NODE_model_update_interval,
                          i_episode=None):
        fit = updates % NODE_model_update_interval == 0 and self.task.fit_due(i_episode)
        nb = min(NODE_memory.position or len(NODE_memory), 32768) if fit else 0
        fit = fit and nb > 0
        if hasattr(memory, "sample_rows"):
            ws = self._workspace(batch_size)
            eps_ready = self._noise is None and getattr(memory, "device_rng", False)
            memory.sample_rows(batch_size, out=ws.mb, **({"eps_out": ws.eps} if eps_ready else {}))
            if fit:
                self.fit_node_rows(NODE_memory.sample_rows(nb) if hasattr(NODE_memory, "sample_rows") else
                                   self._rows_from_host(NODE_memory.sample(batch_size=nb)).to(self.device))
            return self.update_on_device(ws, updates, eps_ready=eps_ready)
        batch = memory.sample(batch_size=batch_size)
        node_rows = NODE_memory.sample(batch_size=nb) if fit else None
        return self.update_from_host(batch, updates, node_rows)

    def _rows_from_host(self, batch):
        lay = self.lay
        batch = tuple(batch)
        sig = None
        if lay.sig is not None:
            sig, batch = batch[4], batch[:4] + batch[5:]
        state, action, reward, constraint, lya_in, next_lya_in, nstate, mask = batch[:8]
        n = np.asarray(state).shape[0]
        host = np.zeros((n, lay.LD), dtype=np.float32)
        if sig is not None:
            host[:, lay.sig] = sig
        host[:, lay.obs:lay.obs + lay.obs_dim] = state
        host[:, lay.act:lay.act + lay.act_dim] = np.asarray(action).reshape(n, lay.act_dim)
        host[:, lay.rew], host[:, lay.con] = reward, constraint
        host[:, lay.lya:lay.lya + lay.lya_dim] = lya_in
        host[:, lay.nlya:lay.nlya + lay.lya_dim] = next_lya_in
        host[:, lay.nobs:lay.nobs + lay.obs_dim] = nstate
        host[:, lay.mask] = mask
        if len(batch) > 9 and batch[8] is not None and np.asarray(batch[8]).dtype != object:
            host[:, lay.t], host[:, lay.nt] = batch[8], batch[9]
        return torch.from_numpy(host)

    def update_from_host(self, batch, updates, node_batch=None):
        B = np.asarray(batch[0]).shape[0]
        ws = self._workspace(B)
        ws.mb.copy_(self._rows_from_host(batch), non_blocking=False)
        if node_batch is not None:
            if len(node_batch) <= 4:
                o, a_, no = node_batch[:3]
                n = np.asarray(o).shape[0]
                t = np.asarray(node_batch[3]).reshape(n) if len(node_batch) == 4 else np.zeros(n)
                zl = np.zeros((n, self.lay.lya_dim))
                node_batch = (o, a_, np.zeros(n), np.zeros(n)) + ((np.zeros(n),) if self.lay.sig is not None else ()) \
                    + (zl, zl, no, np.ones(n), t, t)
            self.fit_node_rows(self._rows_from_host(node_batch).to(self.device))
        return self.update_on_device(ws, updates)

    def _workspace(self, B):
        if B not in self._ws:
            self._ws[B] = _Workspace(B, self.hidden, self.device, self.lay, self.task)
        return self._ws[B]

    def fit_node_rows(self, rows):
        self._fit(*self.task.fit_inputs(rows))

    def _fit(self, p_obs, obs_ld, action, p_nobs, nobs_ld, N):
        task = self.task
        self._fill.clear()
        if N not in self._fit_ws:
            while len(self._fit_ws) >= 2:
                self._fit_ws.pop(next(iter(self._fit_ws)))
            w = task.fit_ws(N)
            w.update(graphs=GraphCache(task.solvers), warm=0)
            self._fit_ws[N] = w
        w = self._fit_ws[N]
        w["u"].copy_(action)
        key = (p_obs, obs_ld, p_nobs, nobs_ld, self.solver)
        part1 = lambda: task.fit_part1(w, p_obs, obs_ld, p_nobs, nobs_ld, N)
        if not self._graphs_on() or w["warm"] < 1:
            w["warm"] += 1
            part1()
            self._fit_part2(w, N, task.fit_solver.forward_finish())
            return
        g = w["graphs"]
        g.replay(("p1",) + key, part1)
        if self.solver == "dopri5" and not task.fit_solver.first_step_done():
            self._fit_part2(w, N, task.fit_solver.forward_finish())
            return
        g.replay(("p2",) + key, lambda: self._fit_part2(w, N, task.fit_solver.forward_finish(assume_single_step=True)))

    def _fit_part2(self, w, N, pred):
        s = stream_ptr()
        ns = self.task.n_s
        nblk = (N + 255) // 256
        NG = N * self.world
        _lib.call("nlbac_mse_fwd_bwd", pred.data_ptr(), ns, w["nst"].data_ptr(), ns, N, NG, ns, w["dpred"].data_ptr(),
                  ns, w["part"].data_ptr(), s)
        _lib.call("nlbac_sum_partials", w["part"].data_ptr(), nblk, 1, 1.0 / (NG * ns),
                  self.sc.data_ptr() + 4 * SC.SC_NODE_LOSS, s)
        self.task.fit_solver.backward(w["dpred"], need_du=False, need_params=True)
        n_steps = max(1, len(self.task.fit_solver.ctx.get("steps") or [None]))
        used = self.task.fit_solver.accumulate_param_grads(
            self.ar_n, max(1, min(self.n_fit_slabs, self.ar_n.n_slabs // min(n_steps, self.ar_n.n_slabs))))
        self._adam(self.ar_n, 1e-3, used, extra=self.sc[SC.SC_NODE_LOSS:SC.SC_NODE_LOSS + 1])

    def _plan(self, ws, NP=None):
        NP = NP or self.task.n_pol
        return ws.plan.get(NP) or ws.plan.setdefault(NP, Plan(self, ws, NP))

    def auglag_fused(self, ws, P, lam_upd):
        if self.world > 1:
            return None, None, None
        P.auglag.do_lambda_update, P.auglag.do_backup_lambda_update = lam_upd, ws.blam_upd
        return C.byref(P.auglag), self._tickets.data_ptr() + 4 * 12, self.sc.data_ptr()

    def auglag(self, ws, n_cbf, lam_upd):
        s, call = stream_ptr(), _lib.call
        NP = ws.np_now
        if self.world == 1:
            ws.p_part_q, ws.n_part_q = ws.part_q.data_ptr(), ws.nblk
            return
        ncol = n_cbf + 1 + (n_cbf if NP == 2 else 0)
        xs = self._exchange_buf("sums", 64)
        call("nlbac_sum_partials", ws.part_c.data_ptr(), ws.nblk, ncol, 1.0, xs.data_ptr(), s)
        for pp in range(NP):
            call("nlbac_sum_partials", ws.part_q[pp].data_ptr(), ws.nblk, 2, 1.0, xs.data_ptr() + 4 * (32 + 2 * pp), s)
        self.dp.all_reduce_(xs)
        ws.p_part_q, ws.n_part_q = xs.data_ptr() + 4 * 32, 1
        call("nlbac_auglag", xs.data_ptr(), 1, n_cbf, 1, float(self.batch_size), lam_upd, ws.blam_upd,
             self.task.ratio_mode, self.task.backup_mode if NP == 2 else 0, self.task.lam_lo, self.task.lam_hi,
             self.sc.data_ptr(), s)

    def update_on_device(self, ws, updates, sync=True, eps_ready=False, prefetch=None):
        pre, ws._prefetched = ws._prefetched, None
        if prefetch is not None:
            eps_ready = True
            if pre is None or pre[0] != updates:
                pre = None
                prefetch()
        else:
            pre = None
        ws._pre_now, ws._prefetch_fn, ws._sync = pre, prefetch, sync
        if self._noise is not None:
            assert len(self._noise) == self.task.n_eps, "set_noise needs %d draws" % self.task.n_eps
            order = self.task.eps_order or range(self.task.n_eps)
            for i, j in enumerate(order):
                ws.eps[i].copy_(self._noise[j].to(self.device).reshape(ws.eps[i].shape))
            self._noise = None
        elif not eps_ready:
            ws.eps.normal_()
        soft = (updates % self.target_update_interval == 0)
        lam_upd = 1 if updates % self.Lagrangian_multiplier_update_interval == 0 else 0
        NP = ws.np_now = self.task.n_pol_now(updates)
        ws.updates_now = updates
        assert ws._pre_now is None or ws._pre_now[1] == NP
        ws.blam_upd = self.task.backup_lam_due(updates, self.Lagrangian_multiplier_update_interval)
        self._readback.choose_mirror(sync, self.world == 1 and not self._graphs_on() and self.fold_launches)
        if not self._graphs_on() or ws.warm < 1:
            ws.warm += 1
            self._upd_part1(ws, soft)
            self._upd_part2(ws, lam_upd, False)
        else:
            g = ws.graphs
            k1, k2 = ("p1", soft, self.solver, NP), ("p2", lam_upd, ws.blam_upd, self.solver, NP)
            g.replay(k1, lambda: self._upd_part1(ws, soft))
            if self.solver == "dopri5" and not self.task.first_step_done():
                self._upd_part2(ws, lam_upd, False)
            else:
                g.replay(k2, lambda: self._upd_part2(ws, lam_upd, True))
        h = self._readback.returns(sync)
        if h is None:
            return None
        alpha_loss = float(h[SC.SC_ALOSS]) if self.automatic_entropy_tuning else 0.0
        return (float(h[SC.SC_QF1]), float(h[SC.SC_QF2]), float(h[SC.SC_LF]), float(h[SC.SC_PL1]),
                alpha_loss, float(h[SC.SC_ALPHA]))

    def _upd_part1(self, ws, soft):
        B, A = ws.B, self.lay.act_dim
        G = B * self.world
        s = stream_ptr()
        NP = ws.np_now
        P = self._plan(ws, NP)
        LD = P.LD

        if ws._pre_now is None:
            self._policy_forward(ws, P, NP)
        self.task.rollout_begin(ws, P)
        self._fill = collections.deque((lambda: self._part1_targets(ws, P, B, G, LD, s),
                                        lambda: self._part1_critic_step(ws, P, B, soft),
                                        lambda: self._part1_actor_q(ws, P, B, G, NP, s)))
        self._fill_first = self.task.rollout_waits == 1
        if ws._pre_now is not None and ws._pre_now[2]:
            self._fill.popleft()
        if self.solver != "dopri5" or torch.cuda.is_current_stream_capturing():
            self.drain_fill()

    def _policy_forward(self, ws, P, NP):
        B, A = ws.B, self.lay.act_dim
        s, call = stream_ptr(), _lib.call
        if self.fold_launches:
            assert P.head_pol3 is not None
            call("nlbac_mlp_fwd_gauss", P.n_pol3, P.io_pol3, 1 + NP, B, C.byref(P.head_pol3), s)
        else:
            pol = self.policy
            call("nlbac_mlp_fwd", P.n_pol3, P.io_pol3, 1 + NP, B, s)
            call("nlbac_gauss_sample_fwd", ws.heads3.data_ptr(), 2 * A, ws.eps.data_ptr(), pol.action_scale.data_ptr(),
                 pol.action_bias.data_ptr(), A, (1 + NP) * B, ws.act3.data_ptr(), A, ws.logp3.data_ptr(), s)

    def _prefetch_next(self, ws, updates):
        fn = ws._prefetch_fn
        if fn is None or self._graphs_on() or self.world != 1 or self._noise is not None:
            return
        if ws._sync and self._readback.mirror is None:
            return
        fn()
        NP = self.task.n_pol_now(updates + 1)
        ws._prefetched = (updates + 1, NP, self._prefetch_launches(ws, NP))

    def update_prefetch(self, ws, updates, prefetch):
        if self._graphs_on() or self.world != 1:
            return
        prefetch()
        NP = self.task.n_pol_now(updates)
        ws._prefetched = (updates, NP, self._prefetch_launches(ws, NP))

    def _prefetch_launches(self, ws, NP):
        P = self._plan(ws, NP)
        self._policy_forward(ws, P, NP)
        if self.task.rollout_waits >= 3:
            return False
        self._part1_targets(ws, P, ws.B, ws.B * self.world, P.LD, stream_ptr())
        return True

    def _fill_one(self):
        k, self._fill_first = (2 if self._fill_first else 1), False
        while k and self._fill:
            self._fill.popleft()()
            k -= 1

    def drain_fill(self):
        while self._fill:
            self._fill.popleft()()

    def _part1_targets(self, ws, P, B, G, LD, s):
        sc, call = self.sc.data_ptr(), _lib.call
        one = self.world == 1
        call("nlbac_mlp_fwd", P.n_six, P.io_six, P.n_six_count, B, s)
        q = ws.q6
        if one and len(self.h_extra) <= 1 and self.fold_launches:
            assert P.head_td is not None
            call("nlbac_mlp_bwd_data_head", P.n_crit, P.io_crit, len(self.h_crit), B, C.byref(P.head_td), s)
            return
        call("nlbac_td_targets", q[0].data_ptr(), q[1].data_ptr(), q[2].data_ptr(), ws.nlogp.data_ptr(),
             P.p_rew, P.p_con, P.p_mask, LD, q[3].data_ptr(), q[4].data_ptr(), q[5].data_ptr(),
             sc + 4 * SC.SC_ALPHA, self.gamma, B, G, ws.dq3[0].data_ptr(), ws.dq3[1].data_ptr(), ws.dq3[2].data_ptr(),
             ws.next_q.data_ptr(), ws.next_l.data_ptr(), ws.part_td.data_ptr(),
             *((self._tickets.data_ptr(), 1.0 / G, sc + 4 * SC.SC_QF1) if one else (None, 0.0, None)), s)
        if not one:
            call("nlbac_sum_partials", ws.part_td.data_ptr(), ws.nblk, 3, 1.0 / G, sc + 4 * SC.SC_QF1, s)
        for k in range(len(self.h_extra)):
            call("nlbac_td_value", q[6 + 2 * k].data_ptr(), ws.mb.data_ptr() + 4 * self.lay.sig, LD, P.p_mask, LD,
                 q[7 + 2 * k].data_ptr(), self.gamma, B, G, ws.dq3[3 + k].data_ptr(), None, ws.part_tdx[k].data_ptr(),
                 *((self._tickets.data_ptr() + 4 * (1 + k), 1.0 / G, sc + 4 * SC.SC_XLOSS) if one else (None, 0.0, None)), s)
            if not one:
                call("nlbac_sum_partials", ws.part_tdx[k].data_ptr(), ws.nblk, 1, 1.0 / G, sc + 4 * SC.SC_XLOSS, s)

        call("nlbac_mlp_bwd_data", P.n_crit, P.io_crit, len(self.h_crit), B, s)

    def _part1_critic_step(self, ws, P, B, soft):
        a = self.ar_c
        bwd_weights(P.n_crit, P.io_crit, len(self.h_crit), B, a.n_slabs, a.n, self.device, ws=P.sk_crit)
        self._adam(a, self.critic_lyapunov_lr, a.n_slabs, extra=self.sc[SC.SC_QF1:SC.SC_QF1 + 3],
                   target=a.target.data_ptr(), tau=self.tau if soft else -1.0)

    def _part1_actor_q(self, ws, P, B, G, NP, s):
        sc, call = self.sc.data_ptr(), _lib.call
        call("nlbac_mlp_fwd", P.n_q5, P.io_q5, P.n_q5_count, B, s)
        if self.world == 1 and self.fold_launches:
            return
        fused = ticket = None
        if self.world == 1:
            assert P.actor_scalars is not None
            fused, ticket = C.byref(P.actor_scalars), self._tickets.data_ptr() + 4 * 8
        call("nlbac_actor_q_terms", ws.qpi[0].data_ptr(), ws.qpi[1].data_ptr(), ws.logp2.data_ptr(),
             sc + 4 * SC.SC_ALPHA, B, G, NP, ws.dq_pi[0].data_ptr(), ws.dq_pi[1].data_ptr(), ws.part_q.data_ptr(), fused, ticket, s)

    def _upd_part2(self, ws, lam_upd, assume_single):
        B, A, Do = ws.B, self.lay.act_dim, self.lay.obs_dim
        G = B * self.world
        s = stream_ptr()
        NP = ws.np_now
        P = self._plan(ws, NP)
        sc, call = self.sc.data_ptr(), _lib.call
        ws.q5_bwd_done = False
        du2, du_ld = self.task.loss_and_backward(ws, P, lam_upd, assume_single)

        if ws.q5_bwd_done:
            pass
        elif self.world == 1 and self.fold_launches:
            assert P.head_actor_q is not None
            call("nlbac_mlp_bwd_data_head", P.n_q5, P.io_q5, 2 * NP, B, C.byref(P.head_actor_q), s)
        else:
            call("nlbac_mlp_bwd_data", P.n_q5, P.io_q5, 2 * NP, B, s)
        if self.fold_launches:
            H = P.head_gauss
            assert H is not None
            H.da[2], H.da_ld[2] = du2.data_ptr(), du_ld
            job = P.cf_job
            F = H.finish[2]
            F.kind = 4 if job else 0
            if job:
                F.partials, F.sc = job[4], job[3]
            call("nlbac_mlp_bwd_data_head", P.n_act, P.io_act, NP, B, C.byref(H), s)
        else:
            D = Do + A
            call("nlbac_gauss_sample_bwd", ws.heads2.data_ptr(), 2 * A, ws.eps[1:1 + NP].data_ptr(),
                 self.policy.action_scale.data_ptr(), A, NP * B, B, ws.dxq[0].data_ptr() + 4 * Do, D, ws.dxq[1].data_ptr() + 4 * Do,
                 D, du2.data_ptr(), du_ld, sc + 4 * SC.SC_ALPHA, 1.0 / G, ws.dheads2.data_ptr(), 2 * A, s)
            call("nlbac_mlp_bwd_data", P.n_act, P.io_act, NP, B, s)
        tune = self.automatic_entropy_tuning
        p_part_q, n_part = ws.p_part_q, ws.n_part_q
        for g, cnt, nets, gio, sk_ws in P.act_groups:
            a = g.arena
            bwd_weights(nets, gio, cnt, B, a.n_slabs, a.n, self.device, ws=sk_ws)
            la = a.theta.data_ptr() + 4 * g.la_off

            def alpha_grads(p_grad, g=g, cnt=cnt, la=la):
                if self.world > 1:
                    call("nlbac_actor_scalars", p_part_q, n_part, G, g.first, cnt, self.target_entropy, la, g.la_stride,
                         p_grad + 4 * g.la_off, sc, s)
                if not tune:
                    z = torch.zeros(1, device=self.device)
                    for off in [g.la_off + k * g.la_stride for k in range(cnt)]:
                        call("nlbac_axpby", 0.0, z.data_ptr(), 0.0, None, 1, p_grad + 4 * off, s)
            refresh = ([g.la_off + k * g.la_stride for k in range(cnt)],
                       [sc + 4 * (SC.SC_ALPHA + g.first + k) for k in range(cnt)]) if tune else None
            last = g is P.act_groups[-1][0]
            mir = self._readback.mirror if last else None
            self._adam(a, self.lr, a.n_slabs, before_step=alpha_grads, alpha=refresh, mirror=mir[1] if mir else None)
            if mir:
                self._readback.mirrored(mir[0])
        self._prefetch_next(ws, ws.updates_now)

    def save_model(self, output):
        print('Saving models in {}'.format(output))
        torch.save(self.policy.state_dict(), '{}/actor.pkl'.format(output))
        torch.save(self.critic.state_dict(), '{}/critic.pkl'.format(output))
        torch.save(self.lyapunovNet.state_dict(), '{}/lyapunov.pkl'.format(output))
        if self.BarrierNet is not None:
            torch.save(self.BarrierNet.state_dict(), '{}/barrier.pkl'.format(output))
        torch.save(self.neural_ode_model.state_dict(), '{}/node_model.pkl'.format(output))

    def load_weights(self, output):
        if output is None:
            return
        print('Loading models from {}'.format(output))
        dev = torch.device(self.device)
        self.policy.load_state_dict(torch.load('{}/actor.pkl'.format(output), map_location=dev, weights_only=True))
        self.critic.load_state_dict(torch.load('{}/critic.pkl'.format(output), map_location=dev, weights_only=True))
        self.lyapunovNet.load_state_dict(torch.load('{}/lyapunov.pkl'.format(output), map_location=dev, weights_only=True))
        if self.BarrierNet is not None:
            self.BarrierNet.load_state_dict(torch.load('{}/barrier.pkl'.format(output), map_location=dev, weights_only=True))
        self.repack_all()

    def load_model(self, actor_path, critic_path, lyapunov_path, barrier_path=None):
        if actor_path is not None:
            self.policy.load_state_dict(torch.load(actor_path, weights_only=True))
        if critic_path is not None:
            self.critic.load_state_dict(torch.load(critic_path, weights_only=True))
        if lyapunov_path is not None:
            self.lyapunovNet.load_state_dict(torch.load(lyapunov_path, weights_only=True))
        if barrier_path is not None and self.BarrierNet is not None:
            self.BarrierNet.load_state_dict(torch.load(barrier_path, weights_only=True))
        self.repack_all()


    def save_checkpoint(self, path):
        names = ("ar_c", "ar_a", "ar_b", "ar_n")
        state = {"solver": self.solver, "sc": self.sc.cpu()}
        for n in names:
            a = getattr(self, n, None)
            if a is not None:
                state[n] = {k: getattr(a, k).cpu() for k in ("theta", "m", "v", "state")}
                if a.target is not None:
                    state[n]["target"] = a.target.cpu()
        torch.save(state, path)

    def load_checkpoint(self, path):
        state = torch.load(path, map_location="cpu", weights_only=True)
        for n, a_state in state.items():
            if n in ("solver", "sc"):
                continue
            a = getattr(self, n)
            for k, v in a_state.items():
                getattr(a, k).copy_(v)
        self.sc.copy_(state["sc"])
        self.solver = state["solver"]
        self.repack_all()


class _TargetView:

    def __init__(self, module, arena):
        self.module, self.arena = module, arena

    def state_dict(self):
        out = {}
        for k, p in self.module.named_parameters():
            off = self.arena.offset_of[id(p)]
            out[k] = self.arena.target[off:off + p.numel()].view(p.shape)
        return out

    def load_state_dict(self, sd):
        cur = self.state_dict()
        with torch.no_grad():
            for k, v in sd.items():
                cur[k].copy_(v)
```

Before: 3.702 million samples/s.

## Fuse replay sampling into held actor Adam step and precompute Adam constants

The last actor Adam step is now held and launched together with the next replay-batch draw in one fused kernel. Leading blocks sample rows while the remaining blocks run Adam, which removes a separate launch and lets the two overlap. Adam bias-correction constants for the next step are precomputed by block 0 into an extended state, so other blocks no longer need a per-block thread-0 pow computation and barrier. Slab gradient loads, scatter-table entries and the target value are software-prefetched one iteration ahead. The cost is more register pressure and harder ordering logic between the held step and the prefetch path.

```diff
diff --git a/include/nlbac_hip.h b/include/nlbac_hip.h
--- a/include/nlbac_hip.h
+++ b/include/nlbac_hip.h
@@ -86,6 +86,15 @@
                      const long *alpha_off, float *const *alpha_dst,
                      const float *mirror_src, float *mirror_dst ,
                      int n_mirror, nlbac_stream_t s);
+typedef struct nlbac_draw {
+    const float *src; long src_rows; int ld; long n_rows; float *dst; float *eps; long n_eps;
+    unsigned long long seed, draw;
+} nlbac_draw;
+int nlbac_adam_fused_draw(float *p, float *m, float *v, const float *grad, int n_slabs, long slab_stride, long n,
+                          void *state, double lr, float *target, float tau, const void *scatter,
+                          const void *scatter_target, int scatter_slots, int n_alpha, const long *alpha_off,
+                          float *const *alpha_dst, const float *mirror_src, float *mirror_dst, int n_mirror,
+                          const nlbac_draw *draw, nlbac_stream_t s);
 int nlbac_reduce_slabs(float *out, const float *grad, int n_slabs, long slab_stride, long n, nlbac_stream_t s);
 int nlbac_soft_update(float *target, const float *src, long n, float tau, nlbac_stream_t s);
 
diff --git a/neural-ordinary-differential-equations-based-lyapunov-barrier-actor-critic-nlbac_amd/_lib.py b/neural-ordinary-differential-equations-based-lyapunov-barrier-actor-critic-nlbac_amd/_lib.py
--- a/neural-ordinary-differential-equations-based-lyapunov-barrier-actor-critic-nlbac_amd/_lib.py
+++ b/neural-ordinary-differential-equations-based-lyapunov-barrier-actor-critic-nlbac_amd/_lib.py
@@ -113,6 +113,11 @@
                 ("x", C.c_void_p)]
 
 
+class Draw(C.Structure):
+    _fields_ = [("src", C.c_void_p), ("src_rows", C.c_long), ("ld", C.c_int), ("n_rows", C.c_long), ("dst", C.c_void_p),
+                ("eps", C.c_void_p), ("n_eps", C.c_long), ("seed", C.c_uint64), ("draw", C.c_uint64)]
+
+
 _P, _I, _F, _D, _L = C.c_void_p, C.c_int, C.c_float, C.c_double, C.c_long
 
 _PROTOS = {
@@ -134,6 +139,8 @@
     "nlbac_adam_step": [_P, _P, _P, _P, _I, _L, _L, _P, _P, _F, _P],
     "nlbac_adam_fused": [_P, _P, _P, _P, _I, _L, _L, _P, _D, _P, _F, _P, _P, _I, _I, C.POINTER(C.c_long),
                          C.POINTER(C.c_void_p), _P, _P, _I, _P],
+    "nlbac_adam_fused_draw": [_P, _P, _P, _P, _I, _L, _L, _P, _D, _P, _F, _P, _P, _I, _I, C.POINTER(C.c_long),
+                              C.POINTER(C.c_void_p), _P, _P, _I, C.POINTER(Draw), _P],
     "nlbac_node_rk_mask_words": [C.POINTER(Mlp), C.POINTER(Mlp), _I],
     "nlbac_concat_adj_in": [_P, _I, _P, _I, _I, _P, _I, _P, _P, _P],
     "nlbac_concat_adj_out": [_P, _P, _I, _I, _P, _I, _I, _P, _P],
diff --git a/neural-ordinary-differential-equations-based-lyapunov-barrier-actor-critic-nlbac_amd/arena.py b/neural-ordinary-differential-equations-based-lyapunov-barrier-actor-critic-nlbac_amd/arena.py
--- a/neural-ordinary-differential-equations-based-lyapunov-barrier-actor-critic-nlbac_amd/arena.py
+++ b/neural-ordinary-differential-equations-based-lyapunov-barrier-actor-critic-nlbac_amd/arena.py
@@ -4,6 +4,9 @@
 
 from . import _lib
 from ._lib import MAX_LAYERS, Mlp, MlpIO
+
+
+STATE_WORDS = 12
 
 
 def _align4(n):
@@ -39,7 +42,7 @@
         self.m = torch.zeros(n, dtype=torch.float32, device=dev)
         self.v = torch.zeros(n, dtype=torch.float32, device=dev)
         self.target = torch.zeros(n, dtype=torch.float32, device=dev) if self.with_target else None
-        self.state = torch.zeros(4, dtype=torch.int32, device=dev)
+        self.state = torch.zeros(STATE_WORDS, dtype=torch.int32, device=dev)
         self.offset_of = {}
         with torch.no_grad():
             for p, off in self._pending:
diff --git a/neural-ordinary-differential-equations-based-lyapunov-barrier-actor-critic-nlbac_amd/csrc/optim_kernels.hip b/neural-ordinary-differential-equations-based-lyapunov-barrier-actor-critic-nlbac_amd/csrc/optim_kernels.hip
--- a/neural-ordinary-differential-equations-based-lyapunov-barrier-actor-critic-nlbac_amd/csrc/optim_kernels.hip
+++ b/neural-ordinary-differential-equations-based-lyapunov-barrier-actor-critic-nlbac_amd/csrc/optim_kernels.hip
@@ -11,25 +11,38 @@
     float step_size;
     float bc2_sqrt;
     unsigned ticket;
+    struct Consts {
+        double bc1;
+        float bc2_sqrt;
+        int step;
+    } next[2];
 };
+static_assert(sizeof(AdamState) == 48, "arena.py allocates AdamState as 12 int32");
+
+__device__ __forceinline__ double adam_bc1(int t) { return 1.0 - pow(0.9, (double)t); }
+__device__ __forceinline__ float adam_bc2_sqrt(int t) { return (float)sqrt(1.0 - pow(0.999, (double)t)); }
 
 __global__ void adam_prepare_kernel(AdamState* st, double lr) {
     if (threadIdx.x == 0 && blockIdx.x == 0) {
         const int t = st->step + 1;
         st->step = t;
-        const double bc1 = 1.0 - pow(0.9, (double)t);
-        const double bc2 = 1.0 - pow(0.999, (double)t);
-        st->step_size = (float)(lr / bc1);
-        st->bc2_sqrt = (float)sqrt(bc2);
+        st->step_size = (float)(lr / adam_bc1(t));
+        st->bc2_sqrt = adam_bc2_sqrt(t);
     }
 }
 
 __device__ __forceinline__ float adam_one(float& p, float& m, float& v, float g, float step_size, float bc2_sqrt) {
-    m = m + (g - m) * (float)(1.0 - 0.9);
-    v = v * 0.999f + ((float)(1.0 - 0.999) * g) * g;
+#pragma clang fp contract(off)
+    m = fmaf(g - m, (float)(1.0 - 0.9), m);
+    v = fmaf(g, (float)(1.0 - 0.999) * g, v * 0.999f);
     const float denom = sqrtf(v) / bc2_sqrt + 1e-8f;
     p = p + ((-step_size) * m) / denom;
     return p;
+}
+
+__device__ __forceinline__ float polyak_one(float t, float p, float tau) {
+#pragma clang fp contract(off)
+    return fmaf(tau, p, t * (1.0f - tau));
 }
 
 __global__ __launch_bounds__(256) void adam_step_kernel(float* __restrict__ p, float* __restrict__ m,
@@ -58,8 +71,8 @@
         reinterpret_cast<float4*>(v)[i] = vv;
         if (target) {
             float4 t = reinterpret_cast<float4*>(target)[i];
-            t.x = t.x * (1.0f - tau) + pp.x * tau; t.y = t.y * (1.0f - tau) + pp.y * tau;
-            t.z = t.z * (1.0f - tau) + pp.z * tau; t.w = t.w * (1.0f - tau) + pp.w * tau;
+            t.x = polyak_one(t.x, pp.x, tau); t.y = polyak_one(t.y, pp.y, tau);
+            t.z = polyak_one(t.z, pp.z, tau); t.w = polyak_one(t.w, pp.w, tau);
             reinterpret_cast<float4*>(target)[i] = t;
         }
     }
@@ -69,7 +82,7 @@
         float pp = p[i], mm = m[i], vv = v[i];
         adam_one(pp, mm, vv, g, step_size, bc2_sqrt);
         p[i] = pp; m[i] = mm; v[i] = vv;
-        if (target) target[i] = target[i] * (1.0f - tau) + pp * tau;
+        if (target) target[i] = polyak_one(target[i], pp, tau);
     }
 }
 
@@ -84,25 +97,56 @@
 }
 #define scatter2 scatter_n<SLOTS>
 
-__device__ __forceinline__ float4 slab_sum4(const float* __restrict__ grad, int n_slabs, long slab_stride, long i) {
-    float4 g = reinterpret_cast<const float4*>(grad)[i];
-    int s = 1;
-    for (; s + 3 < n_slabs; s += 4) {
-        const float4 a = reinterpret_cast<const float4*>(grad + (long)s * slab_stride)[i];
-        const float4 b = reinterpret_cast<const float4*>(grad + (long)(s + 1) * slab_stride)[i];
-        const float4 c = reinterpret_cast<const float4*>(grad + (long)(s + 2) * slab_stride)[i];
-        const float4 d = reinterpret_cast<const float4*>(grad + (long)(s + 3) * slab_stride)[i];
-        g.x += a.x; g.y += a.y; g.z += a.z; g.w += a.w;
-        g.x += b.x; g.y += b.y; g.z += b.z; g.w += b.w;
-        g.x += c.x; g.y += c.y; g.z += c.z; g.w += c.w;
-        g.x += d.x; g.y += d.y; g.z += d.z; g.w += d.w;
-    }
-    for (; s < n_slabs; ++s) {
-        const float4 a = reinterpret_cast<const float4*>(grad + (long)s * slab_stride)[i];
-        g.x += a.x; g.y += a.y; g.z += a.z; g.w += a.w;
-    }
-    return g;
-}
+template <int SLOTS>
+struct ScatEntries {
+    ulonglong2 e[4][SLOTS / 2];
+    __device__ __forceinline__ void load(const unsigned long long* __restrict__ scat, long i) {
+        const ulonglong2* q = reinterpret_cast<const ulonglong2*>(scat) + i * (4 * (SLOTS / 2));
+#pragma unroll
+        for (int j = 0; j < 4; ++j)
+#pragma unroll
+            for (int k = 0; k < SLOTS / 2; ++k) e[j][k] = q[j * (SLOTS / 2) + k];
+    }
+    __device__ __forceinline__ void store(int j, float val) const {
+#pragma unroll
+        for (int k = 0; k < SLOTS / 2; ++k) {
+            if (e[j][k].x) *reinterpret_cast<float*>(e[j][k].x) = val;
+            if (e[j][k].y) *reinterpret_cast<float*>(e[j][k].y) = val;
+        }
+    }
+};
+
+#define ADAM_SLAB_BATCH 8
+struct SlabBatch {
+    float4 g[ADAM_SLAB_BATCH];
+    __device__ __forceinline__ void load(const float* __restrict__ grad, int n_slabs, long slab_stride, long i) {
+#pragma unroll
+        for (int s = 0; s < ADAM_SLAB_BATCH; ++s)
+            if (s < n_slabs) g[s] = reinterpret_cast<const float4*>(grad + (long)s * slab_stride)[i];
+    }
+    __device__ __forceinline__ float4 sum(const float* __restrict__ grad, int n_slabs, long slab_stride, long i) const {
+        float4 a = g[0];
+#pragma unroll
+        for (int s = 1; s < ADAM_SLAB_BATCH; ++s)
+            if (s < n_slabs) { a.x += g[s].x; a.y += g[s].y; a.z += g[s].z; a.w += g[s].w; }
+        int s = ADAM_SLAB_BATCH;
+        for (; s + 3 < n_slabs; s += 4) {
+            const float4 b = reinterpret_cast<const float4*>(grad + (long)s * slab_stride)[i];
+            const float4 c = reinterpret_cast<const float4*>(grad + (long)(s + 1) * slab_stride)[i];
+            const float4 d = reinterpret_cast<const float4*>(grad + (long)(s + 2) * slab_stride)[i];
+            const float4 e = reinterpret_cast<const float4*>(grad + (long)(s + 3) * slab_stride)[i];
+            a.x += b.x; a.y += b.y; a.z += b.z; a.w += b.w;
+            a.x += c.x; a.y += c.y; a.z += c.z; a.w += c.w;
+            a.x += d.x; a.y += d.y; a.z += d.z; a.w += d.w;
+            a.x += e.x; a.y += e.y; a.z += e.z; a.w += e.w;
+        }
+        for (; s < n_slabs; ++s) {
+            const float4 b = reinterpret_cast<const float4*>(grad + (long)s * slab_stride)[i];
+            a.x += b.x; a.y += b.y; a.z += b.z; a.w += b.w;
+        }
+        return a;
+    }
+};
 
 struct AlphaRefresh { long off[2]; float* dst[2]; const float* mirror_src; float* mirror_dst; int n_mirror; };
 __device__ __forceinline__ void alpha_refresh(const AlphaRefresh& AR, long e, float p_new) {
@@ -118,33 +162,72 @@
         }
 }
 
-template <int SLOTS>
+struct DrawRider {
+    const float4* src; int ld4; long n_rows, src_rows; float4* dst; float* eps; long n_eps;
+    unsigned long long seed, draw; unsigned n_blocks;
+};
+__device__ __forceinline__ void sample_rows_body(long t, const float4* __restrict__ src, int ld4, long n_rows,
+                                                 long src_rows, float4* __restrict__ dst, float* __restrict__ eps,
+                                                 long n_eps, unsigned long long seed, unsigned long long draw);
+
+template <int SLOTS, bool DRAW>
 __global__ __launch_bounds__(256) void adam_fused_kernel(float* __restrict__ p, float* __restrict__ m,
                                                          float* __restrict__ v, const float* __restrict__ grad,
                                                          int n_slabs, long slab_stride, long n, AdamState* st, double lr,
                                                          float* __restrict__ target, float tau,
                                                          const unsigned long long* __restrict__ scat,
                                                          const unsigned long long* __restrict__ scat_t,
-                                                         const AlphaRefresh AR) {
-    __shared__ float s_const[2];
-    __shared__ int s_step;
-    if (threadIdx.x == 0) {
-        const int t = __hip_atomic_load(&st->step, __ATOMIC_RELAXED, __HIP_MEMORY_SCOPE_AGENT) + 1;
-        const double bc1 = 1.0 - pow(0.9, (double)t);
-        const double bc2 = 1.0 - pow(0.999, (double)t);
-        s_const[0] = (float)(lr / bc1);
-        s_const[1] = (float)sqrt(bc2);
-        s_step = t;
-    }
-    __syncthreads();
-    const float step_size = s_const[0], bc2_sqrt = s_const[1];
+                                                         const AlphaRefresh AR, const DrawRider DR) {
+    constexpr auto RLX = __ATOMIC_RELAXED;
+    constexpr auto AGENT = __HIP_MEMORY_SCOPE_AGENT;
+    if (blockIdx.x == 0) {
+        if (threadIdx.x == 0) {
+            const int t2 = __hip_atomic_load(&st->step, RLX, AGENT) + 2;
+            AdamState::Consts& c = st->next[t2 & 1];
+            c.bc1 = adam_bc1(t2);
+            c.bc2_sqrt = adam_bc2_sqrt(t2);
+            c.step = t2;
+        }
+        return;
+    }
+    const unsigned n_draw = DRAW ? DR.n_blocks : 0u;
+    if (DRAW && blockIdx.x <= n_draw) {
+        sample_rows_body((long)(blockIdx.x - 1) * 256 + threadIdx.x, DR.src, DR.ld4, DR.n_rows, DR.src_rows, DR.dst,
+                         DR.eps, DR.n_eps, DR.seed, DR.draw);
+        return;
+    }
+    const unsigned bid = blockIdx.x - n_draw - 1, n_blk = gridDim.x - n_draw - 1;
     const long n4 = n >> 2;
-    const long stride = (long)gridDim.x * blockDim.x;
-    for (long i = (long)blockIdx.x * blockDim.x + threadIdx.x; i < n4; i += stride) {
-        float4 g = slab_sum4(grad, n_slabs, slab_stride, i);
-        float4 pp = reinterpret_cast<float4*>(p)[i];
-        float4 mm = reinterpret_cast<float4*>(m)[i];
-        float4 vv = reinterpret_cast<float4*>(v)[i];
+    const long stride = (long)n_blk * blockDim.x;
+    long i = (long)bid * blockDim.x + threadIdx.x;
+    const bool have = i < n4;
+    SlabBatch G;
+    ScatEntries<SLOTS> S, St;
+    float4 pp, mm, vv, tt;
+    if (have) {
+        pp = reinterpret_cast<float4*>(p)[i];
+        mm = reinterpret_cast<float4*>(m)[i];
+        vv = reinterpret_cast<float4*>(v)[i];
+        G.load(grad, n_slabs, slab_stride, i);
+        if (target) tt = reinterpret_cast<float4*>(target)[i];
+        if (scat) S.load(scat, i);
+        if (target && scat_t) St.load(scat_t, i);
+    }
+    const int t = __hip_atomic_load(&st->step, RLX, AGENT) + 1;
+    const int c_step[2] = {__hip_atomic_load(&st->next[0].step, RLX, AGENT), __hip_atomic_load(&st->next[1].step, RLX, AGENT)};
+    const double c_bc1[2] = {__hip_atomic_load(&st->next[0].bc1, RLX, AGENT), __hip_atomic_load(&st->next[1].bc1, RLX, AGENT)};
+    const float c_bc2[2] = {__hip_atomic_load(&st->next[0].bc2_sqrt, RLX, AGENT),
+                            __hip_atomic_load(&st->next[1].bc2_sqrt, RLX, AGENT)};
+    float step_size, bc2_sqrt;
+    if (c_step[t & 1] == t) {
+        step_size = (float)(lr / c_bc1[t & 1]);
+        bc2_sqrt = c_bc2[t & 1];
+    } else {
+        step_size = (float)(lr / adam_bc1(t));
+        bc2_sqrt = adam_bc2_sqrt(t);
+    }
+    while (i < n4) {
+        float4 g = G.sum(grad, n_slabs, slab_stride, i);
         adam_one(pp.x, mm.x, vv.x, g.x, step_size, bc2_sqrt);
         adam_one(pp.y, mm.y, vv.y, g.y, step_size, bc2_sqrt);
         adam_one(pp.z, mm.z, vv.z, g.z, step_size, bc2_sqrt);
@@ -156,22 +239,26 @@
             alpha_refresh(AR, 4 * i + 0, pp.x); alpha_refresh(AR, 4 * i + 1, pp.y);
             alpha_refresh(AR, 4 * i + 2, pp.z); alpha_refresh(AR, 4 * i + 3, pp.w);
         }
-        if (scat) {
-            scatter2(scat, 4 * i + 0, pp.x); scatter2(scat, 4 * i + 1, pp.y);
-            scatter2(scat, 4 * i + 2, pp.z); scatter2(scat, 4 * i + 3, pp.w);
-        }
+        if (scat) { S.store(0, pp.x); S.store(1, pp.y); S.store(2, pp.z); S.store(3, pp.w); }
         if (target) {
-            float4 t = reinterpret_cast<float4*>(target)[i];
-            t.x = t.x * (1.0f - tau) + pp.x * tau; t.y = t.y * (1.0f - tau) + pp.y * tau;
-            t.z = t.z * (1.0f - tau) + pp.z * tau; t.w = t.w * (1.0f - tau) + pp.w * tau;
-            reinterpret_cast<float4*>(target)[i] = t;
-            if (scat_t) {
-                scatter2(scat_t, 4 * i + 0, t.x); scatter2(scat_t, 4 * i + 1, t.y);
-                scatter2(scat_t, 4 * i + 2, t.z); scatter2(scat_t, 4 * i + 3, t.w);
-            }
-        }
-    }
-    for (long i = (n4 << 2) + (long)blockIdx.x * blockDim.x + threadIdx.x; i < n; i += stride) {
+            float4 t4 = tt;
+            t4.x = polyak_one(t4.x, pp.x, tau); t4.y = polyak_one(t4.y, pp.y, tau);
+            t4.z = polyak_one(t4.z, pp.z, tau); t4.w = polyak_one(t4.w, pp.w, tau);
+            reinterpret_cast<float4*>(target)[i] = t4;
+            if (scat_t) { St.store(0, t4.x); St.store(1, t4.y); St.store(2, t4.z); St.store(3, t4.w); }
+        }
+        i += stride;
+        if (i < n4) {
+            pp = reinterpret_cast<float4*>(p)[i];
+            mm = reinterpret_cast<float4*>(m)[i];
+            vv = reinterpret_cast<float4*>(v)[i];
+            G.load(grad, n_slabs, slab_stride, i);
+            if (target) tt = reinterpret_cast<float4*>(target)[i];
+            if (scat) S.load(scat, i);
+            if (target && scat_t) St.load(scat_t, i);
+        }
+    }
+    for (long i = (n4 << 2) + (long)bid * blockDim.x + threadIdx.x; i < n; i += stride) {
         float g = grad[i];
         for (int s = 1; s < n_slabs; ++s) g += grad[s * slab_stride + i];
         float pp = p[i], mm = m[i], vv = v[i];
@@ -180,9 +267,9 @@
         alpha_refresh(AR, i, pp);
         if (scat) scatter2(scat, i, pp);
         if (target) {
-            const float t = target[i] * (1.0f - tau) + pp * tau;
-            target[i] = t;
-            if (scat_t) scatter2(scat_t, i, t);
+            const float tg = polyak_one(target[i], pp, tau);
+            target[i] = tg;
+            if (scat_t) scatter2(scat_t, i, tg);
         }
     }
     __syncthreads();
@@ -190,11 +277,11 @@
     if (threadIdx.x == 0) {
         s_is_last = 0;
         const unsigned ticket = __hip_atomic_fetch_add(&st->ticket, 1u, __ATOMIC_RELAXED, __HIP_MEMORY_SCOPE_AGENT);
-        if (ticket == gridDim.x - 1) {
+        if (ticket == n_blk - 1) {
             __hip_atomic_store(&st->ticket, 0u, __ATOMIC_RELAXED, __HIP_MEMORY_SCOPE_AGENT);
             st->step_size = step_size;
             st->bc2_sqrt = bc2_sqrt;
-            __hip_atomic_store(&st->step, s_step, __ATOMIC_RELAXED, __HIP_MEMORY_SCOPE_AGENT);
+            __hip_atomic_store(&st->step, t, __ATOMIC_RELAXED, __HIP_MEMORY_SCOPE_AGENT);
             s_is_last = 1;
         }
     }
@@ -271,11 +358,11 @@
     return 0;
 }
 
-extern "C" int nlbac_adam_fused(float* p, float* m, float* v, const float* grad, int n_slabs, long slab_stride, long n,
-                                void* state, double lr, float* target, float tau, const void* scatter,
-                                const void* scatter_target, int scatter_slots, int n_alpha, const long* alpha_off,
-                                float* const* alpha_dst, const float* mirror_src, float* mirror_dst, int n_mirror,
-                                nlbac_stream_t s) {
+extern "C" int nlbac_adam_fused_draw(float* p, float* m, float* v, const float* grad, int n_slabs, long slab_stride,
+                                     long n, void* state, double lr, float* target, float tau, const void* scatter,
+                                     const void* scatter_target, int scatter_slots, int n_alpha, const long* alpha_off,
+                                     float* const* alpha_dst, const float* mirror_src, float* mirror_dst, int n_mirror,
+                                     const nlbac_draw* draw, nlbac_stream_t s) {
     NLBAC_REQUIRE(p && m && v && grad && state, "nlbac_adam_fused: null pointer");
     NLBAC_REQUIRE(scatter_slots == 2 || scatter_slots == 4 || (!scatter && !scatter_target),
                   "nlbac_adam_fused: scatter tables hold 2 or 4 slots per parameter");
@@ -290,15 +377,41 @@
     }
     NLBAC_REQUIRE(n_slabs >= 1 && n >= 1 && lr > 0.0, "nlbac_adam_fused: bad sizes");
     NLBAC_REQUIRE(((uintptr_t)p | (uintptr_t)m | (uintptr_t)v | (uintptr_t)grad | (uintptr_t)target) % 16 == 0 &&
-                      slab_stride % 4 == 0 && ((uintptr_t)scatter | (uintptr_t)scatter_target) % 8 == 0,
+                      slab_stride % 4 == 0 && ((uintptr_t)scatter | (uintptr_t)scatter_target) % 16 == 0,
                   "nlbac_adam_fused: buffers must be 16-byte aligned");
     NLBAC_REQUIRE(!scatter_target || (target && tau >= 0.f), "nlbac_adam_fused: scatter_target without a target");
-    hipLaunchKernelGGL((scatter_slots == 4 ? adam_fused_kernel<4> : adam_fused_kernel<2>), dim3(stream_grid(n, 4)), dim3(256),
+    DrawRider DR = {};
+    if (draw) {
+        NLBAC_REQUIRE(draw->src && draw->dst && draw->src_rows >= 1 && draw->src_rows < (1L << 32) && draw->n_rows >= 1 &&
+                          draw->n_eps >= 0,
+                      "nlbac_adam_fused_draw: bad draw arguments");
+        NLBAC_REQUIRE(draw->ld >= 4 && draw->ld % 4 == 0 && ((uintptr_t)draw->src % 16) == 0 && ((uintptr_t)draw->dst % 16) == 0,
+                      "nlbac_adam_fused_draw: rows must be whole float4s (ld %d)", draw->ld);
+        NLBAC_REQUIRE(draw->eps || draw->n_eps == 0, "nlbac_adam_fused_draw: n_eps without a buffer");
+        const long total = draw->n_rows * (draw->ld / 4), q = (draw->n_eps + 3) / 4;
+        const long blocks = ((total > q ? total : q) + 255) / 256;
+        NLBAC_REQUIRE(blocks < (1L << 30), "nlbac_adam_fused_draw: draw too large for one launch");
+        DR.src = (const float4*)draw->src; DR.ld4 = draw->ld / 4; DR.n_rows = draw->n_rows; DR.src_rows = draw->src_rows;
+        DR.dst = (float4*)draw->dst; DR.eps = draw->eps; DR.n_eps = draw->n_eps; DR.seed = draw->seed; DR.draw = draw->draw;
+        DR.n_blocks = (unsigned)blocks;
+    }
+    hipLaunchKernelGGL((scatter_slots == 4 ? (draw ? adam_fused_kernel<4, true> : adam_fused_kernel<4, false>)
+                                           : (draw ? adam_fused_kernel<2, true> : adam_fused_kernel<2, false>)),
+                       dim3(1 + DR.n_blocks + stream_grid(n, 4)), dim3(256),
                        0, (hipStream_t)s, p, m, v, grad, n_slabs, slab_stride, n, (AdamState*)state, lr,
                        (tau >= 0.f) ? target : nullptr, tau, (const unsigned long long*)scatter,
-                       (const unsigned long long*)scatter_target, AR);
+                       (const unsigned long long*)scatter_target, AR, DR);
     NLBAC_CHECK_LAUNCH("nlbac_adam_fused");
     return 0;
+}
+
+extern "C" int nlbac_adam_fused(float* p, float* m, float* v, const float* grad, int n_slabs, long slab_stride, long n,
+                                void* state, double lr, float* target, float tau, const void* scatter,
+                                const void* scatter_target, int scatter_slots, int n_alpha, const long* alpha_off,
+                                float* const* alpha_dst, const float* mirror_src, float* mirror_dst, int n_mirror,
+                                nlbac_stream_t s) {
+    return nlbac_adam_fused_draw(p, m, v, grad, n_slabs, slab_stride, n, state, lr, target, tau, scatter, scatter_target,
+                                 scatter_slots, n_alpha, alpha_off, alpha_dst, mirror_src, mirror_dst, n_mirror, nullptr, s);
 }
 
 extern "C" int nlbac_reduce_slabs(float* out, const float* grad, int n_slabs, long slab_stride, long n, nlbac_stream_t s) {
@@ -364,11 +477,9 @@
 
 __device__ __forceinline__ float u01(unsigned x) { return (float)(x >> 8) * 0x1p-24f + 0x1p-25f; }
 
-__global__ __launch_bounds__(256) void sample_rows_kernel(const float4* __restrict__ src, int ld4, long n_rows,
-                                                          long src_rows, float4* __restrict__ dst,
-                                                          float* __restrict__ eps, long n_eps,
-                                                          unsigned long long seed, unsigned long long draw) {
-    const long t = (long)blockIdx.x * 256 + threadIdx.x;
+__device__ __forceinline__ void sample_rows_body(long t, const float4* __restrict__ src, int ld4, long n_rows,
+                                                 long src_rows, float4* __restrict__ dst, float* __restrict__ eps,
+                                                 long n_eps, unsigned long long seed, unsigned long long draw) {
     const uint2 key = make_uint2((unsigned)seed, (unsigned)(seed >> 32));
     if (t < n_rows * ld4) {
         const long r = t / ld4;
@@ -388,6 +499,13 @@
         for (int k = 0; k < 4; ++k)
             if (4 * t + k < n_eps) eps[4 * t + k] = v[k];
     }
+}
+
+__global__ __launch_bounds__(256) void sample_rows_kernel(const float4* __restrict__ src, int ld4, long n_rows,
+                                                          long src_rows, float4* __restrict__ dst,
+                                                          float* __restrict__ eps, long n_eps,
+                                                          unsigned long long seed, unsigned long long draw) {
+    sample_rows_body((long)blockIdx.x * 256 + threadIdx.x, src, ld4, n_rows, src_rows, dst, eps, n_eps, seed, draw);
 }
 
 extern "C" int nlbac_sample_rows(const float* src, long src_rows, int ld, long n_rows, float* dst, float* eps,
diff --git a/neural-ordinary-differential-equations-based-lyapunov-barrier-actor-critic-nlbac_amd/sac_cbf_clf/held_step.py b/neural-ordinary-differential-equations-based-lyapunov-barrier-actor-critic-nlbac_amd/sac_cbf_clf/held_step.py
--- /dev/null
+++ b/neural-ordinary-differential-equations-based-lyapunov-barrier-actor-critic-nlbac_amd/sac_cbf_clf/held_step.py
@@ -0,0 +1,36 @@
+import ctypes as C
+
+from .. import _lib
+
+
+def due(prefetch_fn, graphs_on, world, noise_pending, sync, mirror):
+    if prefetch_fn is None or graphs_on or world != 1 or noise_pending:
+        return False
+    if sync and mirror is None:
+        return False
+    return True
+
+
+class HeldStep:
+    def __init__(self):
+        self.args = None
+
+    def hold(self, args):
+        assert self.args is None, "an optimiser step is already held"
+        self.args = tuple(args)
+
+    def take(self):
+        args, self.args = self.args, None
+        return args
+
+    def flush(self, stream):
+        args = self.take()
+        if args is not None:
+            _lib.call("nlbac_adam_fused", *args, stream)
+
+
+def launch_draw(held, draw, stream):
+    if held is None:
+        _lib.call("nlbac_sample_rows", *draw, stream)
+    else:
+        _lib.call("nlbac_adam_fused_draw", *held, C.byref(_lib.Draw(*draw)), stream)
diff --git a/neural-ordinary-differential-equations-based-lyapunov-barrier-actor-critic-nlbac_amd/sac_cbf_clf/replay_memory.py b/neural-ordinary-differential-equations-based-lyapunov-barrier-actor-critic-nlbac_amd/sac_cbf_clf/replay_memory.py
--- a/neural-ordinary-differential-equations-based-lyapunov-barrier-actor-critic-nlbac_amd/sac_cbf_clf/replay_memory.py
+++ b/neural-ordinary-differential-equations-based-lyapunov-barrier-actor-critic-nlbac_amd/sac_cbf_clf/replay_memory.py
@@ -109,14 +109,17 @@
         import torch
         from .. import _lib
         from ..arena import stream_ptr
+        from .held_step import launch_draw
         self.flush()
         if out is None:
             out = torch.empty(batch_size, self.lay.LD, dtype=torch.float32, device=self.device)
         if self.device_rng:
             self._draws += 1
-            _lib.call("nlbac_sample_rows", self.rows.data_ptr(), self._len, self.lay.LD, batch_size, out.data_ptr(),
-                      eps_out.data_ptr() if eps_out is not None else None,
-                      eps_out.numel() if eps_out is not None else 0, self._seed, self._draws, stream_ptr())
+            held = getattr(self.agent, "held_step", None)
+            launch_draw(held.take() if held is not None else None,
+                        (self.rows.data_ptr(), self._len, self.lay.LD, batch_size, out.data_ptr(),
+                         eps_out.data_ptr() if eps_out is not None else None,
+                         eps_out.numel() if eps_out is not None else 0, self._seed, self._draws), stream_ptr())
             return out
         idx = torch.tensor(random.sample(range(self._len), batch_size), dtype=torch.int64).to(self.device)
         _lib.call("nlbac_gather_rows", self.rows.data_ptr(), self._len, self.lay.LD, idx.data_ptr(), batch_size,
diff --git a/neural-ordinary-differential-equations-based-lyapunov-barrier-actor-critic-nlbac_amd/sac_cbf_clf/sac_cbf_clf.py b/neural-ordinary-differential-equations-based-lyapunov-barrier-actor-critic-nlbac_amd/sac_cbf_clf/sac_cbf_clf.py
--- a/neural-ordinary-differential-equations-based-lyapunov-barrier-actor-critic-nlbac_amd/sac_cbf_clf/sac_cbf_clf.py
+++ b/neural-ordinary-differential-equations-based-lyapunov-barrier-actor-critic-nlbac_amd/sac_cbf_clf/sac_cbf_clf.py
@@ -11,6 +11,7 @@
 from .. import _lib
 from ..arena import Arena, bwd_weights, pack, stream_ptr
 from . import _layout as SC
+from .held_step import HeldStep, due as held_step_due
 from .model import BarrierNetwork, GaussianPolicy, LyaNetwork, QNetwork
 from .scalars_readback import ScalarsReadback
 from .tasks import TASKS
@@ -155,6 +156,7 @@
         self._tickets = torch.zeros(16, dtype=torch.int32, device=dev)
         self._ws = {}
         self._noise = None
+        self.held_step = HeldStep()
         self._fit_ws = {}
         self._fill = collections.deque()
         self._fill_first = True
@@ -212,7 +214,8 @@
             self._xb[name] = torch.zeros(n, dtype=torch.float32, device=self.device)
         return self._xb[name]
 
-    def _adam(self, arena, lr, n_slabs, extra=None, target=None, tau=-1.0, before_step=None, alpha=None, mirror=None):
+    def _adam(self, arena, lr, n_slabs, extra=None, target=None, tau=-1.0, before_step=None, alpha=None, mirror=None,
+              hold=False):
         s = stream_ptr()
         a = arena
         scat, scat_t = a.scatter_tables()
@@ -223,10 +226,14 @@
         if self.world == 1:
             if before_step is not None:
                 before_step(a.grad.data_ptr())
-            _lib.call("nlbac_adam_fused", a.theta.data_ptr(), a.m.data_ptr(), a.v.data_ptr(), a.grad.data_ptr(),
-                      n_slabs, a.n, a.n, a.state.data_ptr(), lr, target, tau, scat.data_ptr(), scat_t, a.scatter_slots,
-                      n_al, al_off, al_dst, self.sc.data_ptr() if mirror is not None else None,
-                      mirror.data_ptr() if mirror is not None else None, SC.SC_SIZE if mirror is not None else 0, s)
+            args = (a.theta.data_ptr(), a.m.data_ptr(), a.v.data_ptr(), a.grad.data_ptr(),
+                    n_slabs, a.n, a.n, a.state.data_ptr(), lr, target, tau, scat.data_ptr(), scat_t, a.scatter_slots,
+                    n_al, al_off, al_dst, self.sc.data_ptr() if mirror is not None else None,
+                    mirror.data_ptr() if mirror is not None else None, SC.SC_SIZE if mirror is not None else 0)
+            if hold:
+                self.held_step.hold(args)
+            else:
+                _lib.call("nlbac_adam_fused", *args, s)
             return
         n_extra = 0 if extra is None else extra.numel()
         xb = self._exchange_buf("g%d" % id(a), a.n + 4)
@@ -509,13 +516,20 @@
             call("nlbac_gauss_sample_fwd", ws.heads3.data_ptr(), 2 * A, ws.eps.data_ptr(), pol.action_scale.data_ptr(),
                  pol.action_bias.data_ptr(), A, (1 + NP) * B, ws.act3.data_ptr(), A, ws.logp3.data_ptr(), s)
 
-    def _prefetch_next(self, ws, updates):
-        fn = ws._prefetch_fn
-        if fn is None or self._graphs_on() or self.world != 1 or self._noise is not None:
-            return
-        if ws._sync and self._readback.mirror is None:
-            return
-        fn()
+    def _prefetch_due(self, ws):
+        return held_step_due(ws._prefetch_fn, self._graphs_on(), self.world, self._noise is not None, ws._sync,
+                             self._readback.mirror)
+
+    def _prefetch_next(self, ws, updates, mirror_block=None):
+        if not self._prefetch_due(ws):
+            assert self.held_step.args is None
+            return
+        try:
+            ws._prefetch_fn()
+        finally:
+            self.held_step.flush(stream_ptr())
+        if mirror_block is not None:
+            self._readback.mirrored(mirror_block)
         NP = self.task.n_pol_now(updates + 1)
         ws._prefetched = (updates + 1, NP, self._prefetch_launches(ws, NP))
 
@@ -639,10 +653,12 @@
                        [sc + 4 * (SC.SC_ALPHA + g.first + k) for k in range(cnt)]) if tune else None
             last = g is P.act_groups[-1][0]
             mir = self._readback.mirror if last else None
-            self._adam(a, self.lr, a.n_slabs, before_step=alpha_grads, alpha=refresh, mirror=mir[1] if mir else None)
-            if mir:
+            hold = last and self._prefetch_due(ws)
+            self._adam(a, self.lr, a.n_slabs, before_step=alpha_grads, alpha=refresh, mirror=mir[1] if mir else None,
+                       hold=hold)
+            if mir and not hold:
                 self._readback.mirrored(mir[0])
-        self._prefetch_next(ws, ws.updates_now)
+        self._prefetch_next(ws, ws.updates_now, mir[0] if (mir and hold) else None)
 
     def save_model(self, output):
         print('Saving models in {}'.format(output))
@@ -695,7 +711,11 @@
                 continue
             a = getattr(self, n)
             for k, v in a_state.items():
-                getattr(a, k).copy_(v)
+                dst = getattr(a, k)
+                if k == "state" and v.numel() < dst.numel():
+                    dst.zero_()
+                    dst = dst[:v.numel()]
+                dst.copy_(v)
         self.sc.copy_(state["sc"])
         self.solver = state["solver"]
         self.repack_all()
```

Result: no change. 3.726 million samples/s, median of 6 (+0.6%).
